# daooshee/ReReVST-Code

Measured on AMD Instinct MI355X. Metric: stylized frames/sec at 512x512, 1 style, higher is better.
Workload: dtype f32

## Files before the change

### rerevst-code_amd/csrc/conv_f43.h

```cpp
#pragma once
#include "conv_wino.h"

#ifndef F43_ABL
#define F43_ABL 0
#endif
#ifndef F43_SPAN
#define F43_SPAN 28
#endif

typedef float f32x2 __attribute__((ext_vector_type(2)));

struct F43Geo {
    static constexpr int NT = 256;
    static constexpr int NPOS = 36;
    static constexpr int RAW_ROW_BYTES = 4 * 9 * 32;
    static constexpr int RAW_PIECES = 34 * 4 * 9 * 2;
    static constexpr int RAW_IT = (RAW_PIECES + NT - 1) / NT;
    static constexpr int RAW_BYTES = RAW_IT * NT * 16;
    static constexpr int U_BYTES = NPOS * 32 * 8 * 4;
    static constexpr int U_IT = U_BYTES / 16 / NT;
    static constexpr int SMEM = 2 * RAW_BYTES + 2 * U_BYTES + WINO_PAR_BYTES;
};

__device__ __forceinline__ f32x2 p2sub(const f32x2 a, const f32x2 b) {
    f32x2 r;
    asm("v_pk_add_f32 %0, %1, %2 neg_lo:[0,1] neg_hi:[0,1]" : "=v"(r) : "v"(a), "v"(b));
    return r;
}
template <int IMM>
__device__ __forceinline__ f32x2 lds_rd64(unsigned addr) {
    static_assert(IMM >= 0 && IMM < 65536, "ds_read offset is a 16-bit unsigned immediate");
    f32x2 r;
    asm volatile("ds_read_b64 %0, %1 offset:%2" : "=v"(r) : "v"(addr), "i"(IMM));
    return r;
}

template <bool AG>
__device__ __forceinline__ void mfma_acc(f32x4& acc, const float a, const float b) {
    if constexpr (AG) asm volatile("v_mfma_f32_16x16x4_f32 %0, %1, %2, %0" : "+a"(acc) : "v"(a), "v"(b));
    else asm volatile("v_mfma_f32_16x16x4_f32 %0, %1, %2, %0" : "+v"(acc) : "v"(a), "v"(b));
}
template <bool AG>
__device__ __forceinline__ void mfma_zero(f32x4& acc, const float a, const float b) {
    if constexpr (AG) asm volatile("v_mfma_f32_16x16x4_f32 %0, %1, %2, 0" : "=a"(acc) : "v"(a), "v"(b));
    else asm volatile("v_mfma_f32_16x16x4_f32 %0, %1, %2, 0" : "=v"(acc) : "v"(a), "v"(b));
}

constexpr float F43_A = 0.75f, F43_B = 1.5f;
constexpr float F43_A2 = F43_A * F43_A, F43_B2 = F43_B * F43_B, F43_P = F43_A2 * F43_B2, F43_S = F43_A2 + F43_B2;
constexpr float F43_A3 = F43_A2 * F43_A, F43_B3 = F43_B2 * F43_B;
constexpr unsigned f43_bits(float f) { return __builtin_bit_cast(unsigned, f); }

struct F43Tmp { f32x2 a, b, c, f, g; };
struct F43K { unsigned long long b2, a2, p, s, a, b; };
__device__ __forceinline__ F43K f43_load_k() {
    F43K k;
    asm volatile("s_mov_b64 %0, %6\n\ts_mov_b64 %1, %7\n\ts_mov_b64 %2, %8\n\ts_mov_b64 %3, %9\n\ts_mov_b64 %4, %10\n\ts_mov_b64 %5, %11"
                 : "=s"(k.b2), "=s"(k.a2), "=s"(k.p), "=s"(k.s), "=s"(k.a), "=s"(k.b)
                 : "i"(f43_bits(F43_B2)), "i"(f43_bits(F43_A2)), "i"(f43_bits(F43_P)), "i"(f43_bits(F43_S)), "i"(f43_bits(F43_A)), "i"(f43_bits(F43_B)));
    return k;
}
template <bool NEG>
__device__ __forceinline__ void fmak3s(f32x2& r0, f32x2& r1, f32x2& r2, const f32x2 x0, const f32x2 x1, const f32x2 x2,
                                       const f32x2 c0, const f32x2 c1, const f32x2 c2, const unsigned long long ks) {
    if constexpr (NEG)
        asm volatile("v_pk_fma_f32 %0, %4, %3, %7 op_sel_hi:[1,0,1] neg_lo:[0,1,0] neg_hi:[0,1,0]\n\tv_pk_fma_f32 %1, %5, %3, %8 op_sel_hi:[1,0,1] neg_lo:[0,1,0] neg_hi:[0,1,0]\n\t"
                     "v_pk_fma_f32 %2, %6, %3, %9 op_sel_hi:[1,0,1] neg_lo:[0,1,0] neg_hi:[0,1,0]"
                     : "=&v"(r0), "=&v"(r1), "=&v"(r2) : "s"(ks), "v"(x0), "v"(x1), "v"(x2), "v"(c0), "v"(c1), "v"(c2));
    else
        asm volatile("v_pk_fma_f32 %0, %4, %3, %7 op_sel_hi:[1,0,1]\n\tv_pk_fma_f32 %1, %5, %3, %8 op_sel_hi:[1,0,1]\n\tv_pk_fma_f32 %2, %6, %3, %9 op_sel_hi:[1,0,1]"
                     : "=&v"(r0), "=&v"(r1), "=&v"(r2) : "s"(ks), "v"(x0), "v"(x1), "v"(x2), "v"(c0), "v"(c1), "v"(c2));
}
template <int LB, class LineFn>
__device__ __forceinline__ void f43_in3s(LineFn&& L, const F43K& k) {
    F43Tmp t[3];
    using N0 = std::integral_constant<int, LB>; using N1 = std::integral_constant<int, LB + 1>; using N2 = std::integral_constant<int, LB + 2>;
    using I0 = std::integral_constant<int, 0>; using I1 = std::integral_constant<int, 1>; using I2 = std::integral_constant<int, 2>;
    using I3 = std::integral_constant<int, 3>; using I4 = std::integral_constant<int, 4>; using I5 = std::integral_constant<int, 5>;
#define F43_D(J) L(N0{}, I##J{}), L(N1{}, I##J{}), L(N2{}, I##J{})
#define F43_T(M) t[0].M, t[1].M, t[2].M
    fmak3s<true>(F43_T(a), F43_D(2), F43_D(4), k.b2);
    fmak3s<true>(F43_T(b), F43_D(1), F43_D(3), k.b2);
    fmak3s<true>(F43_T(c), F43_D(2), F43_D(4), k.a2);
    fmak3s<true>(F43_T(f), F43_D(1), F43_D(3), k.a2);
    fmak3s<false>(F43_T(g), F43_D(0), F43_D(4), k.p);
    fmak3s<true>(F43_D(0), F43_D(2), F43_T(g), k.s);
    fmak3s<false>(F43_T(g), F43_D(1), F43_D(5), k.p);
    fmak3s<true>(F43_D(5), F43_D(3), F43_T(g), k.s);
    fmak3s<false>(F43_D(1), F43_T(b), F43_T(a), k.a);
    fmak3s<true>(F43_D(2), F43_T(b), F43_T(a), k.a);
    fmak3s<false>(F43_D(3), F43_T(f), F43_T(c), k.b);
    fmak3s<true>(F43_D(4), F43_T(f), F43_T(c), k.b);
#undef F43_D
#undef F43_T
}
__device__ __forceinline__ void f43_out(const f32x2 m0, const f32x2 m1, const f32x2 m2, const f32x2 m3, const f32x2 m4, const f32x2 m5,
                                        f32x2& y0, f32x2& y1, f32x2& y2, f32x2& y3) {
    f32x2 s1, d1, s2, d2;
    unsigned long long ks;
    asm volatile(
        "v_pk_add_f32 %[s1], %[m1], %[m2]\n\t"
        "v_pk_add_f32 %[d1], %[m1], %[m2] neg_lo:[0,1] neg_hi:[0,1]\n\t"
        "v_pk_add_f32 %[s2], %[m3], %[m4]\n\t"
        "v_pk_add_f32 %[d2], %[m3], %[m4] neg_lo:[0,1] neg_hi:[0,1]\n\t"
        "v_pk_add_f32 %[y0], %[m0], %[s1]\n\t"
        "s_mov_b64 %[k], %[ka]\n\t"
        "v_pk_mul_f32 %[y1], %[d1], %[k] op_sel_hi:[1,0]\n\t"
        "s_mov_b64 %[k], %[ka2]\n\t"
        "v_pk_mul_f32 %[y2], %[s1], %[k] op_sel_hi:[1,0]\n\t"
        "s_mov_b64 %[k], %[ka3]\n\t"
        "v_pk_fma_f32 %[y3], %[d1], %[k], %[m5] op_sel_hi:[1,0,1]\n\t"
        "v_pk_add_f32 %[y0], %[y0], %[s2]\n\t"
        "s_mov_b64 %[k], %[kb]\n\t"
        "v_pk_fma_f32 %[y1], %[d2], %[k], %[y1] op_sel_hi:[1,0,1]\n\t"
        "s_mov_b64 %[k], %[kb2]\n\t"
        "v_pk_fma_f32 %[y2], %[s2], %[k], %[y2] op_sel_hi:[1,0,1]\n\t"
        "s_mov_b64 %[k], %[kb3]\n\t"
        "v_pk_fma_f32 %[y3], %[d2], %[k], %[y3] op_sel_hi:[1,0,1]"
        : [y0] "=&v"(y0), [y1] "=&v"(y1), [y2] "=&v"(y2), [y3] "=&v"(y3), [s1] "=&v"(s1), [d1] "=&v"(d1), [s2] "=&v"(s2), [d2] "=&v"(d2), [k] "=&s"(ks)
        : [m0] "v"(m0), [m1] "v"(m1), [m2] "v"(m2), [m3] "v"(m3), [m4] "v"(m4), [m5] "v"(m5),
          [ka] "i"(f43_bits(F43_A)), [ka2] "i"(f43_bits(F43_A2)), [ka3] "i"(f43_bits(F43_A3)),
          [kb] "i"(f43_bits(F43_B)), [kb2] "i"(f43_bits(F43_B2)), [kb3] "i"(f43_bits(F43_B3)));
}

#ifndef P8_PAD
#define P8_PAD 6
#define P8_COL0 4
#endif
template <int EPI, int LAY = 0>
__global__ __launch_bounds__(256, 1) void conv_f43_k(const ConvP p) {
    static_assert(!(EPI & E_RES), "same-resolution residuals are not needed by the layers this kernel serves");
    constexpr bool INP8 = (LAY & 1) != 0, OUTP8 = (LAY & 2) != 0;
    const int WP = p.Wi + 2 + (INP8 ? P8_PAD : 0);
    using G = F43Geo;
    constexpr int ABL = F43_ABL;
    constexpr int RAW_BYTES = G::RAW_BYTES, U_BYTES = G::U_BYTES, NT = G::NT, NPOS = G::NPOS;
    extern __shared__ __attribute__((aligned(16))) char smem[];
    const int tid = threadIdx.x;
    const int wave = __builtin_amdgcn_readfirstlane(tid >> 6);
    const int lane = tid & 63, t = lane & 15, q = lane >> 4;
    const int tr = t >> 3, tc = t & 7;
    const int nchunks = p.Cin >> 3;
    const int n_ntiles = p.Cout >> 5;

    struct Item { int tx, ty, b, nt; };
    Item cur, nxt, dlt;
    {
        const int GD = gridDim.x, w = blockIdx.x;
        int pix, dpix;
        if (p.xcd_slabs) {
            const int PT = (GD >> 3) / n_ntiles;
            pix = (w & 7) * PT + (w >> 3) / n_ntiles; dpix = 8 * PT;
            cur.nt = (w >> 3) % n_ntiles; dlt.nt = 0;
        } else {
            cur.nt = w % n_ntiles; pix = w / n_ntiles;
            dlt.nt = GD % n_ntiles; dpix = GD / n_ntiles;
        }
        cur.tx = pix % p.tiles_x; cur.ty = (pix / p.tiles_x) % p.tiles_y; cur.b = pix / (p.tiles_x * p.tiles_y);
        dlt.tx = dpix % p.tiles_x; dlt.ty = (dpix / p.tiles_x) % p.tiles_y; dlt.b = dpix / (p.tiles_x * p.tiles_y);
    }
    auto advance = [&](const Item& a) {
        Item r = a;
        r.nt += dlt.nt;
        int carry = 0;
        if (r.nt >= n_ntiles) { r.nt -= n_ntiles; carry = 1; }
        r.tx += dlt.tx + carry;
        if (r.tx >= p.tiles_x) { r.tx -= p.tiles_x; r.ty += 1; }
        r.ty += dlt.ty;
        if (r.ty >= p.tiles_y) { r.ty -= p.tiles_y; r.b += 1; }
        r.b += dlt.b;
        return r;
    };
    const size_t img_floats = (size_t)(p.Hi + 2) * WP * p.Cin;
    auto in_of = [&](const Item& a) {
        return p.in + (size_t)a.b * img_floats + (size_t)(((a.ty + p.ty0) * 32) * WP + (a.tx + p.tx0) * 32 + (INP8 ? P8_COL0 - 1 : 0)) * (INP8 ? 8 : p.Cin);
    };
    const size_t plane_floats = (size_t)(p.Hi + 2) * WP * 8;
    auto lim_of = [&](const Item& a) {
        const long rows_left = (long)(p.Hi + 2) - (long)(a.ty + p.ty0) * 32;
        const long n = (rows_left * WP - (long)(a.tx + p.tx0) * 32 - (INP8 ? P8_COL0 - 1 : 0)) * (INP8 ? 8 : p.Cin) * 4;
        return (int)(n > 0x7fffffffL ? 0x7fffffffL : n);
    };
    auto w_of = [&](const Item& a) { return p.wpk + (size_t)a.nt * nchunks * (U_BYTES / 4); };
    int asrc[G::RAW_IT];
#pragma unroll
    for (int it = 0; it < G::RAW_IT; ++it) {
        int e = it * NT + tid;
        if (e >= G::RAW_PIECES) e = 0;
        const int half = e & 1, xd = (e >> 1) % 9, ph = ((e >> 1) / 9) & 3, y = (e >> 1) / 36;
        const int x = 4 * xd + ph, par = (y >> 2) & 1;
        asrc[it] = ((y * WP + x) * (INP8 ? 8 : p.Cin) + 4 * (half ^ par)) * 4;
        if (ABL & 64) asrc[it] = (it * NT + tid) * 16;
    }
    bool have = cur.b < p.B, have_nxt = false;
    const float* in_t = in_of(cur);
    const float* w_t = w_of(cur);
    int lim_t = lim_of(cur);
    const float* in_n = in_t;
    const float* w_n = w_t;
    int lim_n = lim_t;
    auto stage_u = [&](int chunk) {
        char* udst = smem + 2 * RAW_BYTES + (chunk & 1) * U_BYTES;
#pragma unroll
        for (int it = 0; it < G::U_IT; ++it) bufld16(w_t, udst + (it * NT + wave * 64) * 16, tid * 16, chunk * U_BYTES + it * NT * 16);
    };
    auto stage_raw = [&](int chunk) {
        char* rdst = smem + (chunk & 1) * RAW_BYTES;
        const rsrc_t rs = make_rsrc(INP8 ? in_t + chunk * plane_floats : in_t, lim_t);
#pragma unroll
        for (int it = 0; it < G::RAW_IT; ++it) bufld16_rs(rs, rdst + (it * NT + wave * 64) * 16, asrc[it], INP8 ? 0 : chunk * 32);
    };
    char* const par = smem + 2 * RAW_BYTES + 2 * U_BYTES;
    auto stage_params = [&](int ntile, int img) {
        if (wave < 2) {
            const int e = tid;
            const int row = e >> 3, col = (e & 7) * 4;
            const float* src = p.bias;
            int off = ntile * 32 + col;
            const int pb = img * p.par_bstride;
            if (row >= 1 && row <= 4) { src = (EPI & E_NORM1) ? p.n1 : p.bias; off += (EPI & E_NORM1) ? (row - 1) * p.Cout + pb : 0; }
            if (row >= 5 && row <= 8) { src = (EPI & E_NORM2) ? p.n2 : p.bias; off += (EPI & E_NORM2) ? (row - 5) * p.Cout + pb : 0; }
            if (row >= 9) { src = (EPI & E_NORM2) ? p.sty : p.bias; off += (EPI & E_NORM2) ? (row - 9) * p.Cout + pb : 0; }
            if (row > 10) { src = p.bias; off = ntile * 32; }
            glds16(src + off, par + wave * 1024);
        }
    };

    const unsigned lds0 = (unsigned)(size_t)(__attribute__((address_space(3))) char*)smem;
    const int y0 = 8 * wave + 4 * tr;
    const unsigned rawA = lds0 + y0 * G::RAW_ROW_BYTES + tc * 32 + ((q ^ (2 * (tr & 1))) << 3);
    const unsigned rawB = lds0 + y0 * G::RAW_ROW_BYTES + tc * 32 + ((q ^ (2 * ((tr & 1) ^ 1))) << 3);
    const unsigned offU = lds0 + 2 * RAW_BYTES + t * 64 + ((q ^ ((0 - (t >> 2)) & 3)) << 4);

    const unsigned lane_off = (unsigned)(((4 * (q >> 1)) * (p.W + 2) + 16 * (q & 1)) * p.Cout + 2 * t) * 4u;
#ifndef F43_NAG
#define F43_NAG 28
#endif
    constexpr int NAG = F43_NAG;
    f32x4 accA[NAG][2], accV[NPOS - NAG][2];
    int par_ntile = -1, par_img = -1;
    long long tl[6] = {0, 0, 0, 0, 0, 0}, tl_t = 0;
    auto tick = [&](int k) { if (ABL & 16) { const long long n = clock64(); tl[k] += n - tl_t; tl_t = n; } };
    f32x2 v[NPOS];
    f32x4 ur[2][6];
    auto full_transform = [&](f32x2 (&d)[NPOS]) {
        const F43K k = f43_load_k();
        auto col = [&](auto nc, auto jc) -> f32x2& { return d[decltype(nc)::value * 6 + decltype(jc)::value]; };
        auto row = [&](auto nc, auto jc) -> f32x2& { return d[decltype(jc)::value * 6 + decltype(nc)::value]; };
        f43_in3s<0>(col, k);
        f43_in3s<3>(col, k);
        f43_in3s<0>(row, k);
        f43_in3s<3>(row, k);
    };
    auto read_patch_col = [&](auto rbc, auto dxc) {
        constexpr int RB = decltype(rbc)::value, dx = decltype(dxc)::value;
        static_for([&](auto dyc) {
            constexpr int dy = decltype(dyc)::value;
            constexpr int off = RB + dy * G::RAW_ROW_BYTES + (dx & 3) * 288 + (dx >> 2) * 32;
            v[dx * 6 + dy] = lds_rd64<off>(dy < 4 ? rawA : rawB);
        }, std::make_integer_sequence<int, 6>{});
    };
    auto read_u_batch = [&](unsigned ub, auto bc, auto slotc) {
        constexpr int b = decltype(bc)::value, sl = decltype(slotc)::value;
        static_for([&](auto rc) {
            constexpr int r = decltype(rc)::value;
            ur[sl][r] = lds_rd128<(r * 6 + b) * 1024>(ub);
        }, std::make_integer_sequence<int, 6>{});
    };

    auto chunk_body = [&](int c, auto par_c, auto first_c, bool last) {
        constexpr int PAR = decltype(par_c)::value;
        constexpr bool FIRST = decltype(first_c)::value;
        const bool own_u = c + 1 < nchunks, own_r = c + 2 < nchunks;
        const rsrc_t rs_u = make_rsrc(own_u ? w_t : w_n);
        const int rchunk = own_r ? c + 2 : c + 2 - nchunks;
        const rsrc_t rs_r = make_rsrc(INP8 ? (own_r ? in_t : in_n) + rchunk * plane_floats : (own_r ? in_t : in_n), own_r ? lim_t : lim_n);
        const int usoff = own_u ? (c + 1) * U_BYTES : 0;
        const int rsoff = INP8 ? 0 : rchunk * 32;
        char* const udst = smem + 2 * RAW_BYTES + (1 - PAR) * U_BYTES;
        char* const rdst = smem + PAR * RAW_BYTES;
        const unsigned ub = offU + PAR * U_BYTES;
        const unsigned ubn = offU + (1 - PAR) * U_BYTES;
        using RBt = std::integral_constant<int, (1 - PAR) * RAW_BYTES>;
        static_for([&](auto bc) {
            constexpr int b = decltype(bc)::value;
            if constexpr (b <= 1) asm volatile("s_waitcnt lgkmcnt(0)" ::: "memory");
            else if (last) asm volatile("s_waitcnt lgkmcnt(0)" ::: "memory");
            else asm volatile("s_waitcnt lgkmcnt(6)" ::: "memory");
            if constexpr (b < 5) read_u_batch(ub, std::integral_constant<int, b + 1>{}, std::integral_constant<int, (b + 1) & 1>{});
            static_for([&](auto rc) {
                constexpr int r = decltype(rc)::value, pos = r * 6 + b;
                constexpr int step = b * 6 + r;
                auto dma_req = [&](auto nc) {
                    constexpr int n = decltype(nc)::value;
                    if constexpr (n < G::RAW_IT) bufld16_rs(rs_r, rdst + (n * NT + wave * 64) * 16, asrc[n], rsoff);
                    else if constexpr (n < G::RAW_IT + G::U_IT) bufld16_rs(rs_u, udst + ((n - G::RAW_IT) * NT + wave * 64) * 16, tid * 16, usoff + (n - G::RAW_IT) * NT * 16);
                };
                {
                    constexpr int SPAN = F43_SPAN, NREQ = G::RAW_IT + G::U_IT;
                    constexpr int n = (step * NREQ + SPAN - 1) / SPAN;
                    if constexpr (n < NREQ && (n * SPAN) / NREQ == step) { if (!(ABL & 1)) dma_req(std::integral_constant<int, n>{}); }
                }
                if constexpr (r == 3) {
                    if constexpr (b >= 1) { if (!last) read_patch_col(RBt{}, std::integral_constant<int, b - 1>{}); }
                }
                constexpr bool AG = pos < NAG;
                f32x4 (&ac)[2] = *[&]() -> f32x4 (*)[2] { if constexpr (AG) return &accA[pos]; else return &accV[pos - NAG]; }();
                const f32x2 vv = v[b * 6 + r];
                const f32x4 uu = ur[b & 1][r];
                if constexpr (FIRST) { mfma_zero<AG>(ac[0], vv[0], uu[0]); mfma_zero<AG>(ac[1], vv[0], uu[2]); }
                else { mfma_acc<AG>(ac[0], vv[0], uu[0]); mfma_acc<AG>(ac[1], vv[0], uu[2]); }
                mfma_acc<AG>(ac[0], vv[1], uu[1]);
                mfma_acc<AG>(ac[1], vv[1], uu[3]);
            }, std::make_integer_sequence<int, 6>{});
        }, std::make_integer_sequence<int, 6>{});
        if (!last) read_patch_col(RBt{}, std::integral_constant<int, 5>{});
        tick(1);
        if (!(ABL & 2)) asm volatile("s_waitcnt vmcnt(0) lgkmcnt(0)\n\ts_barrier" ::: "memory");
        else asm volatile("s_waitcnt lgkmcnt(0)" ::: "memory");
        tick(3);
        if (!last) {
            read_u_batch(ubn, std::integral_constant<int, 0>{}, std::integral_constant<int, 0>{});
            if (!(ABL & 8)) full_transform(v);
        }
        tick(5);
    };

    auto next_patch = [&]() {
        static_for([&](auto dxc) { read_patch_col(std::integral_constant<int, 0>{}, dxc); }, std::make_integer_sequence<int, 6>{});
        read_u_batch(offU, std::integral_constant<int, 0>{}, std::integral_constant<int, 0>{});
        if (!(ABL & 2)) asm volatile("s_waitcnt lgkmcnt(0)\n\ts_barrier" ::: "memory");
        else asm volatile("s_waitcnt lgkmcnt(0)" ::: "memory");
        if (!(ABL & 8)) full_transform(v);
    };
    if (have) {
        stage_raw(0);
        stage_u(0);
        stage_raw(1);
        stage_params(cur.nt, cur.b);
        par_ntile = cur.nt; par_img = cur.b;
        __syncthreads();
        next_patch();
        __syncthreads();
    }
    if (ABL & 16) tl_t = clock64();
    while (have) {
        const int e_y0 = (cur.ty + p.ty0) * 32, e_x0 = (cur.tx + p.tx0) * 32, e_b = cur.b, e_ntile = cur.nt;
        nxt = advance(cur);
        have_nxt = nxt.b < p.B;
        in_n = have_nxt ? in_of(nxt) : in_t;
        w_n = have_nxt ? w_of(nxt) : w_t;
        lim_n = have_nxt ? lim_of(nxt) : lim_t;
        if (par_ntile != e_ntile || (p.par_bstride != 0 && par_img != e_b)) {
            __syncthreads();
            stage_params(e_ntile, e_b);
            par_ntile = e_ntile; par_img = e_b;
        }
        tick(0);
        chunk_body(0, std::integral_constant<int, 0>{}, std::true_type{}, false);
        chunk_body(1, std::integral_constant<int, 1>{}, std::false_type{}, false);
        for (int c = 2; c < nchunks; c += 2) {
            chunk_body(c, std::integral_constant<int, 0>{}, std::false_type{}, false);
            chunk_body(c + 1, std::integral_constant<int, 1>{}, std::false_type{}, c + 2 == nchunks);
        }
        cur = nxt; have = have_nxt; in_t = in_n; w_t = w_n; lim_t = lim_n;
        asm volatile("s_nop 15\n\ts_nop 7");
        auto ACC = [&](int i, int nb) -> f32x4 { return i < NAG ? accA[i][nb] : accV[i - NAG][nb]; };
        if (ABL & 32) {
            f32x4 s = ACC(0, 0);
#pragma unroll
            for (int i = 0; i < NPOS; ++i)
#pragma unroll
                for (int nb = 0; nb < 2; ++nb) if (i || nb) s += ACC(i, nb);
            if (s[0] + s[1] + s[2] + s[3] == 123.456f) p.out[tid] = s[0];
            if (have) next_patch();
            continue;
        }
        const int mr = q >> 1, mc0 = 4 * (q & 1);
        const int yb = e_y0 + 8 * wave + 4 * mr, xb0 = e_x0 + 4 * mc0;
        constexpr bool POOL = (EPI & E_POOL) != 0;
        const int Ho = POOL ? (p.H >> 1) : p.H, Wo = POOL ? (p.W >> 1) : p.W;
        constexpr int OP = OUTP8 ? P8_PAD : 0;
        char* const sb = OUTP8 ? (char*)(p.out + (size_t)e_b * (size_t)(Ho + 2) * (Wo + 2 + OP) * p.Cout + (size_t)e_ntile * 4 * (size_t)(Ho + 2) * (Wo + 2 + OP) * 8 +
                                         ((size_t)((POOL ? (e_y0 >> 1) + 4 * wave : e_y0 + 8 * wave) + 1) * (Wo + 2 + OP) + (POOL ? (e_x0 >> 1) : e_x0) + P8_COL0) * 8)
                               : (char*)(p.out + (size_t)e_b * (size_t)(Ho + 2) * (Wo + 2) * p.Cout +
                                 ((size_t)((POOL ? (e_y0 >> 1) + 4 * wave : e_y0 + 8 * wave) + 1) * (Wo + 2) + (POOL ? (e_x0 >> 1) : e_x0) + 1) * p.Cout + e_ntile * 32);
        int rowb = (Wo + 2) * p.Cout * 4, pixb = p.Cout * 4;
        unsigned st_off = POOL ? (unsigned)(((2 * mr) * (Wo + 2) + 2 * mc0) * p.Cout + 2 * t) * 4u : lane_off;
        if constexpr (OUTP8) {
            const unsigned plane = (unsigned)(Ho + 2) * (Wo + 2 + OP) * 32u;
            rowb = (Wo + 2 + OP) * 32; pixb = 32;
            st_off = (POOL ? (unsigned)((2 * mr) * (Wo + 2 + OP) + 2 * mc0) : (unsigned)((4 * (q >> 1)) * (p.W + 2 + OP) + 16 * (q & 1))) * 32u + (unsigned)(t >> 2) * plane + (unsigned)(t & 3) * 8u;
        }
        const bool interior = e_y0 + 32 <= p.H && e_x0 + 32 <= p.W;
        const char* const pl = par + 8 * t;
        const f32x2 bias = *(const f32x2*)(pl);
        f32x2 n1m, n1r, n1lo, n1hi, n2m, n2r, n2lo, n2hi, smean, sstd;
        if constexpr ((EPI & E_NORM1) != 0) { n1m = *(const f32x2*)(pl + 128); n1r = *(const f32x2*)(pl + 256); n1lo = *(const f32x2*)(pl + 384); n1hi = *(const f32x2*)(pl + 512); }
        if constexpr ((EPI & E_NORM2) != 0) {
            n2m = *(const f32x2*)(pl + 640); n2r = *(const f32x2*)(pl + 768); n2lo = *(const f32x2*)(pl + 896); n2hi = *(const f32x2*)(pl + 1024);
            smean = *(const f32x2*)(pl + 1152); sstd = *(const f32x2*)(pl + 1280);
        }
        f32x2 rres[4][2][2];
        if constexpr ((EPI & E_RES_UPS) != 0) {
            const float* const res_b = p.res + (size_t)e_b * (size_t)(p.Hr + 2) * (p.Wr + 2) * p.Cout + e_ntile * 32 + 2 * t;
#pragma unroll
            for (int e = 0; e < 4; ++e)
#pragma unroll
                for (int a = 0; a < 2; ++a)
#pragma unroll
                    for (int b2 = 0; b2 < 2; ++b2) {
                        const bool in = (yb + 2 * a < p.H) && (xb0 + 4 * e + 2 * b2 < p.W);
                        const int pix = in ? (((yb >> 1) + a + 1) * (p.Wr + 2) + ((xb0 + 4 * e) >> 1) + b2 + 1) : 0;
                        rres[e][a][b2] = *(const f32x2*)(res_b + (size_t)pix * p.Cout);
                    }
        }
        float lrk = 0.2f;
        asm volatile("" : "+s"(lrk));
        const f32x2 lrk2 = {lrk, lrk};
#pragma unroll
        for (int e = 0; e < 4; ++e) {
            auto PR = [&](int i) -> f32x2 { return f32x2{ACC(i, 0)[e], ACC(i, 1)[e]}; };
            f32x2 T[6][4];
#pragma unroll
            for (int r = 0; r < 6; ++r) {
                f43_out(PR(r * 6 + 0), PR(r * 6 + 1), PR(r * 6 + 2), PR(r * 6 + 3), PR(r * 6 + 4), PR(r * 6 + 5), T[r][0], T[r][1], T[r][2], T[r][3]);
                __builtin_amdgcn_sched_barrier(0);
            }
            f32x2 pool_prev[2];
#pragma unroll
            for (int j = 0; j < 4; ++j) {
                f32x2 o[4];
                f43_out(T[0][j], T[1][j], T[2][j], T[3][j], T[4][j], T[5][j], o[0], o[1], o[2], o[3]);
#pragma unroll
                for (int i = 0; i < 4; ++i) o[i] = o[i] + bias;
                if (EPI & E_RELU) {
#pragma unroll
                    for (int i = 0; i < 4; ++i) o[i] = f32x2{fmaxf(o[i][0], 0.f), fmaxf(o[i][1], 0.f)};
                }
                if (EPI & E_LRELU) {
#pragma unroll
                    for (int i = 0; i < 4; ++i) { const f32x2 s2 = o[i] * lrk2; o[i] = f32x2{fmaxf(o[i][0], s2[0]), fmaxf(o[i][1], s2[1])}; }
                }
                auto norm_clamp = [&](const f32x2 m, const f32x2 r, const f32x2 lo, const f32x2 hi) {
#pragma unroll
                    for (int i = 0; i < 4; ++i) o[i] = p2sub(o[i], m) * r;
#pragma unroll
                    for (int i = 0; i < 4; ++i) o[i] = f32x2{med3(o[i][0], lo[0], hi[0]), med3(o[i][1], lo[1], hi[1])};
                };
                if constexpr ((EPI & E_NORM1) != 0) norm_clamp(n1m, n1r, n1lo, n1hi);
                if constexpr ((EPI & E_RES_UPS) != 0) {
#pragma unroll
                    for (int i = 0; i < 4; ++i) o[i] = o[i] + rres[e][i >> 1][j >> 1];
                }
                if constexpr ((EPI & E_NORM2) != 0) {
                    norm_clamp(n2m, n2r, n2lo, n2hi);
#pragma unroll
                    for (int i = 0; i < 4; ++i) o[i] = __builtin_elementwise_fma(o[i], sstd, smean);
                }
                if constexpr (POOL) {
                    f32x2 m2[2];
#pragma unroll
                    for (int a = 0; a < 2; ++a) m2[a] = f32x2{fmaxf(o[2 * a][0], o[2 * a + 1][0]), fmaxf(o[2 * a][1], o[2 * a + 1][1])};
                    if ((j & 1) == 0) { pool_prev[0] = m2[0]; pool_prev[1] = m2[1]; continue; }
#pragma unroll
                    for (int a = 0; a < 2; ++a) m2[a] = f32x2{fmaxf(m2[a][0], pool_prev[a][0]), fmaxf(m2[a][1], pool_prev[a][1])};
                    char* const dst = sb + (2 * e + (j >> 1)) * pixb + st_off;
                    if (ABL & 4) { if (m2[0][0] == 123.456f) *(float*)dst = m2[0][0] + m2[1][0]; }
                    else if (interior) {
                        *(f32x2*)(dst) = m2[0]; *(f32x2*)(dst + rowb) = m2[1];
                    } else {
#pragma unroll
                        for (int a = 0; a < 2; ++a)
                            if ((yb >> 1) + a < Ho && ((xb0 + 4 * e) >> 1) + (j >> 1) < Wo) *(f32x2*)(dst + a * rowb) = m2[a];
                    }
                } else {
                    char* const dst = sb + (4 * e + j) * pixb + st_off;
                    if (ABL & 4) { if (o[0][0] == 123.456f) *(float*)dst = o[0][0] + o[1][0] + o[2][0] + o[3][0]; }
                    else if (interior) {
#pragma unroll
                        for (int i = 0; i < 4; ++i) *(f32x2*)(dst + i * rowb) = o[i];
                    } else {
#pragma unroll
                        for (int i = 0; i < 4; ++i)
                            if (yb + i < p.H && xb0 + 4 * e + j < p.W) *(f32x2*)(dst + i * rowb) = o[i];
                    }
                }
            }
        }
        tick(4);
        if (have) next_patch();
        tick(5);
    }
    if ((ABL & 16) && lane == 0) {
#pragma unroll
        for (int k = 0; k < 6; ++k) p.dbg[(blockIdx.x * 4 + wave) * 6 + k] = tl[k];
    }
}

__global__ void pack_f43_k(const float* __restrict__ w, float* __restrict__ dst, int Cout, int Cin) {
    const size_t total = (size_t)Cout * Cin * 36;
    for (size_t i = blockIdx.x * (size_t)blockDim.x + threadIdx.x; i < total; i += (size_t)gridDim.x * blockDim.x) {
        size_t r = i;
        const int fl = (int)(r & 3); r >>= 2;
        const int slot = (int)(r & 3); r >>= 2;
        const int row = (int)(r & 15); r >>= 4;
        const int pos = (int)(r % 36); r /= 36;
        const int nchunks = Cin / 8;
        const int chunk = (int)(r % nchunks); r /= nchunks;
        const int n_tile = (int)r;
        const int pair = slot ^ ((0 - (row >> 2)) & 3);
        const int co = n_tile * 32 + 2 * row + (fl >> 1), ci = chunk * 8 + 2 * pair + (fl & 1);
        const float* g = w + ((size_t)co * Cin + ci) * 9;
        const int pr = pos / 6, pc = pos % 6;
        auto G3 = [](int rw, double g0, double g1, double g2) -> double {
            const double A = (double)F43_A, B = (double)F43_B;
            const double pt[5] = {0.0, A, -A, B, -B};
            if (rw == 5) return g2;
            double N = 1.0;
            for (int l = 0; l < 5; ++l) if (l != rw) N *= pt[rw] - pt[l];
            return (g0 + pt[rw] * g1 + pt[rw] * pt[rw] * g2) / N;
        };
        double rowv[3];
#pragma unroll
        for (int kx = 0; kx < 3; ++kx) rowv[kx] = G3(pr, g[0 * 3 + kx], g[1 * 3 + kx], g[2 * 3 + kx]);
        dst[i] = (float)G3(pc, rowv[0], rowv[1], rowv[2]);
    }
}
```

### rerevst-code_amd/csrc/conv_mfma.h

```cpp
#pragma once
#include <hip/hip_runtime.h>
#include <stdint.h>

typedef float f32x16 __attribute__((ext_vector_type(16)));
typedef float f32x4 __attribute__((ext_vector_type(4)));

enum {
    E_RELU = 1,
    E_LRELU = 2,
    E_NORM1 = 4,
    E_RES = 8,
    E_RES_UPS = 16,
    E_NORM2 = 32,
    E_POOL = 64
};

struct ConvP {
    const float* in;
    int Hi, Wi, Cin;
    float* out;
    int H, W, Cout;
    int B;
    int in_bstride0;
    const float* wpk;
    const float* bias;
    const float* n1;
    const float* res;
    int Hr, Wr;
    const float* n2;
    const float* sty;
    int tiles_x, tiles_y;
    int xcd_slabs;
    float* sc_out;
    int ty0, tx0;
    long long* dbg;
    int cstride;
    int cin_slab_step;
    int par_bstride, bias_bstride;
    long long w_bstride;
    int out_p8;
};

template <int BN>
struct WaveCfg {
    static constexpr int WAVES_N = (BN >= 64) ? 2 : 1;
    static constexpr int WAVES_M = 4 / WAVES_N;
    static constexpr int WN_SUB = BN / 32 / WAVES_N;
    static constexpr int WM_SUB = 4 / WAVES_M;
};

__device__ __forceinline__ void glds16(const float* src, char* lds_wave_base) {
    __builtin_amdgcn_global_load_lds((const __attribute__((address_space(1))) void*)src,
                                     (__attribute__((address_space(3))) void*)lds_wave_base, 16, 0, 0);
}

__device__ __forceinline__ void bufld16(const void* base, char* lds_wave_base, int voff, int soff) {
#if defined(__HIP_DEVICE_COMPILE__)
    __amdgpu_buffer_rsrc_t rs = __builtin_amdgcn_make_buffer_rsrc((void*)base, 0, 0x7fffffff, 0x00020000);
    __builtin_amdgcn_raw_ptr_buffer_load_lds(rs, (__attribute__((address_space(3))) void*)lds_wave_base, 16, voff, soff, 0, 0);
#endif
}

#if defined(__HIP_DEVICE_COMPILE__)
typedef __amdgpu_buffer_rsrc_t rsrc_t;
#else
struct rsrc_t {};
#endif
__device__ __forceinline__ rsrc_t make_rsrc(const void* base, int num_records = 0x7fffffff) {
#if defined(__HIP_DEVICE_COMPILE__)
    return __builtin_amdgcn_make_buffer_rsrc((void*)base, 0, num_records, 0x00020000);
#else
    return rsrc_t{};
#endif
}
__device__ __forceinline__ void bufld16_rs(rsrc_t rs, char* lds_wave_base, int voff, int soff) {
#if defined(__HIP_DEVICE_COMPILE__)
    __builtin_amdgcn_raw_ptr_buffer_load_lds(rs, (__attribute__((address_space(3))) void*)lds_wave_base, 16, voff, soff, 0, 0);
#endif
}

template <int BN, int TAPS, int EPI, int ABL = 0, int MSUB = 0, int LD = 1>
__global__ __launch_bounds__(256) void conv_mfma_k(const ConvP p) {
    using WC = WaveCfg<BN>;
    constexpr int WM_SUB = MSUB ? MSUB : WC::WM_SUB;
    constexpr int TROWS = WC::WAVES_M * WM_SUB * 2;
    constexpr int HWD = (TAPS == 1) ? 16 : 18;
    constexpr int HHT = (TAPS == 1) ? TROWS : TROWS + 2;
    constexpr int NPIX = HHT * HWD;
    constexpr int A_ITERS = (NPIX * 4 + 255) / 256;
    constexpr int A_BYTES = A_ITERS * 256 * 16;
    constexpr int B_PIECES = BN * 4;
    constexpr int B_ITERS = (B_PIECES + 255) / 256;
    constexpr int B_BYTES = BN * 64;
    __shared__ __attribute__((aligned(16))) char smem[2 * A_BYTES + 2 * B_BYTES];

    const int tid = threadIdx.x;
    const int wave = __builtin_amdgcn_readfirstlane(tid >> 6);
    const int lane = tid & 63, h = lane >> 5, l31 = lane & 31;
    const int wave_m = wave % WC::WAVES_M, wave_n = wave / WC::WAVES_M;

    int bx = blockIdx.x;
    const int tx = bx % p.tiles_x;
    bx /= p.tiles_x;
    const int ty = bx % p.tiles_y;
    const int b = bx / p.tiles_y;
    const int n_tile = blockIdx.y;
    const int y0 = ty * TROWS, x0 = tx * 16;
    const int nchunks = p.Cin >> 4;

    const float* in_b = p.in + (size_t)(p.in_bstride0 ? b : 0) * (size_t)(p.Hi + 2) * (p.Wi + 2) * p.Cin;
    const int ys = (TAPS == 1) ? y0 : y0 - 1;
    const int xs = (TAPS == 1) ? x0 : x0 - 1;
    int asrc[A_ITERS];
#pragma unroll
    for (int it = 0; it < A_ITERS; ++it) {
        const int e = it * 256 + tid;
        int pp = e >> 2;
        const int qq = e & 3;
        if (pp >= NPIX) pp = 0;
        const int hy = pp / HWD, hx = pp - hy * HWD;
        asrc[it] = (hy * (p.Wi + 2) + hx) * p.Cin + 4 * (qq ^ ((pp >> 2) & 3));
    }
    const float* in_t = in_b + ((size_t)(ys + 1) * (p.Wi + 2) + (xs + 1)) * p.Cin;
    const float* wsrc = p.wpk + (size_t)n_tile * nchunks * TAPS * (BN * 16) + tid * 4;

    const float* w_tile = p.wpk + (size_t)n_tile * nchunks * TAPS * (BN * 16);
    auto stage = [&](int chunk, int tap, int step) {
        char* bdst = smem + 2 * A_BYTES + (step & 1) * B_BYTES;
        const float* wb = wsrc + (size_t)(chunk * TAPS + tap) * (BN * 16);
#pragma unroll
        for (int it = 0; it < B_ITERS; ++it) {
            if (B_PIECES >= 256 || wave * 64 < B_PIECES) {
                if (LD == 1)
                    bufld16(w_tile, bdst + (it * 256 + wave * 64) * 16, tid * 16, (chunk * TAPS + tap) * (BN * 64) + it * 4096);
                else
                    glds16(wb + it * 1024, bdst + (it * 256 + wave * 64) * 16);
            }
        }
        if (tap == 0) {
            char* adst = smem + (chunk & 1) * A_BYTES;
            const float* ab = in_t + chunk * 16;
#pragma unroll
            for (int it = 0; it < A_ITERS; ++it) {
                if (LD == 1)
                    bufld16(in_t, adst + (it * 256 + wave * 64) * 16, asrc[it] * 4, chunk * 64);
                else
                    glds16(ab + asrc[it], adst + (it * 256 + wave * 64) * 16);
            }
        }
    };

    const int r_ = l31 >> 4, c_ = l31 & 15;
    int offB[WC::WN_SUB][2];
#pragma unroll
    for (int ns = 0; ns < WC::WN_SUB; ++ns) {
        const int jj = (wave_n * WC::WN_SUB + ns) * 32 + l31;
#pragma unroll
        for (int g = 0; g < 2; ++g) offB[ns][g] = jj * 64 + ((((2 * g + h) ^ ((jj >> 2) & 3))) << 4);
    }

    f32x16 acc[WM_SUB][WC::WN_SUB];
#pragma unroll
    for (int ms = 0; ms < WM_SUB; ++ms)
#pragma unroll
        for (int ns = 0; ns < WC::WN_SUB; ++ns)
#pragma unroll
            for (int r = 0; r < 16; ++r) acc[ms][ns][r] = 0.f;

    long long t_start = 0, t_loop = 0;
    if (ABL & 16) t_start = clock64();
    stage(0, 0, 0);
    int step = 0;
    for (int chunk = 0; chunk < nchunks; ++chunk) {
        const char* abuf = smem + (chunk & 1) * A_BYTES;
#pragma unroll
        for (int tap = 0; tap < TAPS; ++tap, ++step) {
            if (!(ABL & 2) || step == 0) __syncthreads();
            if (!(ABL & 1)) {
                if (tap + 1 < TAPS)
                    stage(chunk, tap + 1, step + 1);
                else if (chunk + 1 < nchunks)
                    stage(chunk + 1, 0, step + 1);
            }
            const char* bbuf = smem + 2 * A_BYTES + (step & 1) * B_BYTES;
            const int ky = tap / 3, kx = tap - ky * 3;
            int offA[WM_SUB];
#pragma unroll
            for (int ms = 0; ms < WM_SUB; ++ms) {
                const int msg = wave_m * WM_SUB + ms;
                int pp;
                if (TAPS == 1)
                    pp = (2 * msg + r_) * HWD + c_;
                else
                    pp = (2 * msg + r_ + ky) * HWD + c_ + kx;
                offA[ms] = pp * 64 + ((h ^ ((pp >> 2) & 3)) << 4);
            }
#pragma unroll
            for (int g = 0; g < 2; ++g) {
                f32x4 a[WM_SUB], bb[WC::WN_SUB];
#pragma unroll
                for (int ms = 0; ms < WM_SUB; ++ms) a[ms] = *(const f32x4*)(abuf + (offA[ms] ^ (g << 5)));
#pragma unroll
                for (int ns = 0; ns < WC::WN_SUB; ++ns) bb[ns] = *(const f32x4*)(bbuf + offB[ns][g]);
#pragma unroll
                for (int s = 0; s < 4; ++s)
#pragma unroll
                    for (int ms = 0; ms < WM_SUB; ++ms)
#pragma unroll
                        for (int ns = 0; ns < WC::WN_SUB; ++ns)
                            acc[ms][ns] = __builtin_amdgcn_mfma_f32_32x32x2f32(bb[ns][s], a[ms][s], acc[ms][ns], 0, 0, 0);
            }
        }
    }

    if (ABL & 16) t_loop = clock64();
    const int Ho = (EPI & E_POOL) ? (p.H >> 1) : p.H, Wo = (EPI & E_POOL) ? (p.W >> 1) : p.W;
    float* out_b = p.out + (size_t)b * (size_t)(Ho + 2) * (Wo + 2) * p.Cout;
    const float* res_b = nullptr;
    if (EPI & (E_RES | E_RES_UPS)) res_b = p.res + (size_t)b * (size_t)(p.Hr + 2) * (p.Wr + 2) * p.Cout;
#pragma unroll
    for (int ns = 0; ns < WC::WN_SUB; ++ns) {
#pragma unroll
        for (int cg = 0; cg < 4; ++cg) {
            const int co = n_tile * BN + (wave_n * WC::WN_SUB + ns) * 32 + 8 * cg + 4 * h;
            const f32x4 bias = *(const f32x4*)(p.bias + co);
            f32x4 m1, r1, lo1, hi1, m2, r2, lo2, hi2, smean, sstd;
            if (EPI & E_NORM1) {
                m1 = *(const f32x4*)(p.n1 + co); r1 = *(const f32x4*)(p.n1 + p.Cout + co);
                lo1 = *(const f32x4*)(p.n1 + 2 * p.Cout + co); hi1 = *(const f32x4*)(p.n1 + 3 * p.Cout + co);
            }
            if (EPI & E_NORM2) {
                m2 = *(const f32x4*)(p.n2 + co); r2 = *(const f32x4*)(p.n2 + p.Cout + co);
                lo2 = *(const f32x4*)(p.n2 + 2 * p.Cout + co); hi2 = *(const f32x4*)(p.n2 + 3 * p.Cout + co);
                smean = *(const f32x4*)(p.sty + co); sstd = *(const f32x4*)(p.sty + p.Cout + co);
            }
#pragma unroll
            for (int ms = 0; ms < WM_SUB; ++ms) {
                const int msg = wave_m * WM_SUB + ms;
                const int y = y0 + 2 * msg + r_, x = x0 + c_;
                const bool valid = (y < p.H) && (x < p.W);
                f32x4 v;
#pragma unroll
                for (int e = 0; e < 4; ++e) {
                    float t = acc[ms][ns][4 * cg + e] + bias[e];
                    if (EPI & E_RELU) t = fmaxf(t, 0.f);
                    if (EPI & E_LRELU) t = (t >= 0.f) ? t : t * 0.2f;
                    if (EPI & E_NORM1) {
                        t = (t - m1[e]) * r1[e];
                        t = fminf(hi1[e], fmaxf(lo1[e], t));
                    }
                    v[e] = t;
                }
                if (EPI & (E_RES | E_RES_UPS)) {
                    if (valid) {
                        const int ry = (EPI & E_RES_UPS) ? (y >> 1) : y, rx = (EPI & E_RES_UPS) ? (x >> 1) : x;
                        v += *(const f32x4*)(res_b + ((ry + 1) * (p.Wr + 2) + rx + 1) * p.Cout + co);
                    }
                }
                if (EPI & E_NORM2) {
#pragma unroll
                    for (int e = 0; e < 4; ++e) {
                        float t = (v[e] - m2[e]) * r2[e];
                        t = fminf(hi2[e], fmaxf(lo2[e], t));
                        v[e] = t * sstd[e] + smean[e];
                    }
                }
                if (EPI & E_POOL) {
#pragma unroll
                    for (int e = 0; e < 4; ++e) {
                        float t = v[e];
                        t = fmaxf(t, __shfl_xor(t, 1));
                        t = fmaxf(t, __shfl_xor(t, 16));
                        v[e] = t;
                    }
                    const int y2 = (y0 >> 1) + msg, x2 = (x0 + c_) >> 1;
                    if (r_ == 0 && !(c_ & 1) && y2 < Ho && x2 < Wo) {
                        if (ABL & 4) { if (v[0] == 123.456f) out_b[co] = v[0]; }
                        else *(f32x4*)(out_b + ((y2 + 1) * (Wo + 2) + x2 + 1) * p.Cout + co) = v;
                    }
                } else if (valid) {
                    if (ABL & 4) { if (v[0] == 123.456f) out_b[co] = v[0]; }
                    else *(f32x4*)(out_b + ((y + 1) * (p.W + 2) + x + 1) * p.Cout + co) = v;
                }
            }
        }
    }
    if (ABL & 16) {
        const long long t_issued = clock64();
        __builtin_amdgcn_s_waitcnt(0);
        const long long t_end = clock64();
        if (lane == 0) {
            long long* dbg = p.dbg;
            const int wg = (blockIdx.y * gridDim.x + blockIdx.x) * 4 + wave;
            dbg[wg * 4 + 0] = t_start; dbg[wg * 4 + 1] = t_loop; dbg[wg * 4 + 2] = t_issued; dbg[wg * 4 + 3] = t_end;
        }
    }
}
```

### rerevst-code_amd/csrc/conv_ups5.h

```cpp
#pragma once

struct Ups5Tab {
    static constexpr int G2[5][3] = {{2, 0, 0}, {1, 1, 1}, {-1, -1, 1}, {-1, 1, 1}, {0, 0, 2}};
    static constexpr int BT4[4][4] = {{1, 0, -1, 0}, {0, 1, 1, 0}, {0, -1, 1, 0}, {0, -1, 0, 1}};
    static constexpr int AT[4][5] = {{1, 1, 0, -1, 0}, {0, 1, 1, 0, 0}, {0, 1, 0, 1, 0}, {0, 1, -1, 0, 1}};
    static constexpr int DS[5] = {0, 1, 2, 2, 3};
};
template <int T, int R>
constexpr int ups5_coef(int k) { return T == 0 ? Ups5Tab::BT4[R][k] : Ups5Tab::AT[R][k]; }
template <int T, int R, int N>
__device__ __forceinline__ f32x4 ups5_comb(const f32x4 (&x)[N]) {
    constexpr int F = [] { for (int k = 0; k < N; ++k) if (ups5_coef<T, R>(k) == 1) return k; return -1; }();
    static_assert(F >= 0, "every row has a +1 coefficient");
    f32x4 r = x[F];
    static_for([&](auto kc) {
        constexpr int k = decltype(kc)::value;
        constexpr int c = ups5_coef<T, R>(k);
        static_assert(c == 0 || c == 1 || c == -1, "0 / +-1 coefficients");
        if constexpr (k != F && c == 1) r = e4add(r, x[k]);
        else if constexpr (c == -1) r = f4sub(r, x[k]);
    }, std::make_integer_sequence<int, N>{});
    return r;
}

struct Ups5Geo {
    static constexpr int NT = 256, NB = 2;
    static constexpr int NPOS = 29;
    static constexpr int NUB = 26;
    static constexpr int NPIECE = 16;
    static constexpr int HALO = 18, HALF = 18 * 9;
    static constexpr int PIECES = HALO * HALO * 4;
    static constexpr int RAW_IT = (PIECES + NT - 1) / NT;
    static constexpr int RAW_BYTES = RAW_IT * NT * 16;
    static constexpr int U_BYTES = NUB * 32 * 16 * 4;
    static constexpr int U_IT = U_BYTES / 16 / NT;
    static_assert(U_IT * NT * 16 == U_BYTES, "U image is a whole number of LDS-DMA rounds");
    static constexpr int SMEM = 2 * RAW_BYTES + 2 * U_BYTES + WINO_PAR_BYTES;
    static_assert(SMEM <= 160 * 1024, "LDS");
    static constexpr int OCC = 1;
    static constexpr int vidx(int i) { return i < 25 ? Ups5Tab::DS[i % 5] * 4 + Ups5Tab::DS[i / 5] : (i == 25 ? 5 : i == 26 ? 9 : i == 27 ? 6 : 10); }
    static constexpr int issued(int j) { return (j + 2 < NUB ? 2 : 0) + (j < NPIECE ? 1 : 0); }
    static constexpr int younger(int i) {
        return i == 0 ? 2 + issued(0) : i == 1 ? issued(0) + issued(1) : (i - 2 < NPIECE ? 1 : 0) + issued(i - 1) + issued(i);
    }
    static constexpr int col_iter(int dx) { return 4 * dx + 6; }
    static constexpr int row_iter(int r) { return col_iter(3) + 1 + r; }
};
static_assert(Ups5Geo::row_iter(3) < Ups5Geo::NPOS, "next chunk transformed inside the MFMA loop");

template <int EPI, int PERIMG>
__device__ __forceinline__ void conv_ups5_body(const ConvP& p) {
    static_assert(!(EPI & (E_POOL | E_RES | E_RES_UPS | E_NORM2)), "conv1 epilogues only: bias, activation, saved-stat normalise");
    using G = Ups5Geo;
    constexpr int RAW_BYTES = G::RAW_BYTES, U_BYTES = G::U_BYTES, NT = G::NT, NB = G::NB, NPOS = G::NPOS, NUB = G::NUB;
    extern __shared__ __attribute__((aligned(16))) char smem[];
    const int tid = threadIdx.x;
    const int wave = __builtin_amdgcn_readfirstlane(tid >> 6);
    const int lane = tid & 63, t = lane & 15, q = lane >> 4;
    const int tr = t >> 3, tc = t & 7;
    const int tg = wave;
    const int nchunks = p.Cin >> 4;
    const int n_ntiles = p.Cout >> 5;

    struct Item { int tx, ty, b, nt; };
    Item cur, nxt, dlt;
    {
        const int GD = gridDim.x, w = blockIdx.x;
        int pix, dpix;
        if (p.xcd_slabs) {
            const int PT = (GD >> 3) / n_ntiles;
            pix = (w & 7) * PT + (w >> 3) / n_ntiles; dpix = 8 * PT;
            cur.nt = (w >> 3) % n_ntiles; dlt.nt = 0;
        } else {
            cur.nt = w % n_ntiles; pix = w / n_ntiles;
            dlt.nt = GD % n_ntiles; dpix = GD / n_ntiles;
        }
        cur.tx = pix % p.tiles_x; cur.ty = (pix / p.tiles_x) % p.tiles_y; cur.b = pix / (p.tiles_x * p.tiles_y);
        dlt.tx = dpix % p.tiles_x; dlt.ty = (dpix / p.tiles_x) % p.tiles_y; dlt.b = dpix / (p.tiles_x * p.tiles_y);
    }
    auto advance = [&](const Item& a) {
        Item r = a;
        r.nt += dlt.nt;
        int carry = 0;
        if (r.nt >= n_ntiles) { r.nt -= n_ntiles; carry = 1; }
        r.tx += dlt.tx + carry;
        if (r.tx >= p.tiles_x) { r.tx -= p.tiles_x; r.ty += 1; }
        r.ty += dlt.ty;
        if (r.ty >= p.tiles_y) { r.ty -= p.tiles_y; r.b += 1; }
        r.b += dlt.b;
        return r;
    };
    auto in_of = [&](const Item& a) {
        return p.in + (size_t)a.b * (size_t)(p.Hi + 2) * (p.Wi + 2) * p.Cin + (size_t)(((a.ty + p.ty0) * 16) * (p.Wi + 2) + (a.tx + p.tx0) * 16) * p.Cin;
    };
    auto w_of = [&](const Item& a) { return p.wpk + (size_t)a.nt * nchunks * (NUB * 32 * 16); };
    int asrc[G::RAW_IT];
#pragma unroll
    for (int it = 0; it < G::RAW_IT; ++it) {
        const int e = it * NT + tid;
        int P = e >> 2;
        const int qq = e & 3;
        if (P >= G::HALO * G::HALO) P = 0;
        const int hf = P >= G::HALF, rem = P - hf * G::HALF;
        const int hy = rem / 9, hx = 2 * (rem - hy * 9) + hf;
        asrc[it] = ((hy * (p.Wi + 2) + hx) * p.Cin + 4 * (qq ^ ((hx >> 1) & 3))) * 4;
    }
    const int raw_last_num = ((G::RAW_IT - 1) * NT + wave * 64 < G::PIECES) ? 0x7fffffff : 0;
    bool have = cur.b < p.B, have_nxt = false;
    const float* in_t = in_of(cur);
    const float* w_t = w_of(cur);
    const float* in_n = in_t;
    const float* w_n = w_t;
    auto stage_u = [&](int chunk) {
        char* udst = smem + 2 * RAW_BYTES + (chunk & 1) * U_BYTES;
#pragma unroll
        for (int it = 0; it < G::U_IT; ++it) bufld16(w_t, udst + (it * NT + wave * 64) * 16, tid * 16, chunk * U_BYTES + it * NT * 16);
    };
    auto stage_raw = [&](int chunk) {
        char* rdst = smem + (chunk & 1) * RAW_BYTES;
#pragma unroll
        for (int it = 0; it < G::RAW_IT; ++it)
            if (it * NT + wave * 64 < G::PIECES) bufld16(in_t, rdst + (it * NT + wave * 64) * 16, asrc[it], chunk * 64);
    };
    char* const par = smem + 2 * RAW_BYTES + 2 * U_BYTES;
    auto stage_params = [&](int ntile, int img) {
        if (wave < 2) {
            const int e = tid;
            const int row = e >> 3, col = (e & 7) * 4;
            const float* src = p.bias;
            const int pb = PERIMG ? img * p.par_bstride : 0;
            int off = ntile * 32 + col;
            if (row >= 1 && row <= 4) { src = (EPI & E_NORM1) ? p.n1 : p.bias; off = (EPI & E_NORM1) ? ntile * 32 + col + pb + (row - 1) * p.Cout : off; }
            if (row > 4) { src = p.bias; off = ntile * 32; }
            glds16(src + off, par + wave * 1024);
        }
    };

    const unsigned lds0 = (unsigned)(size_t)(__attribute__((address_space(3))) char*)smem;
    unsigned offD[4];
#pragma unroll
    for (int dx = 0; dx < 4; ++dx) {
        const int hy = 4 * tg + 2 * tr, hx = 2 * tc + dx;
        const int P = (hx & 1) * G::HALF + hy * 9 + (hx >> 1);
        offD[dx] = lds0 + P * 64 + ((q ^ ((hx >> 1) & 3)) << 4);
    }
    const unsigned offU = lds0 + 2 * RAW_BYTES + t * 64 + ((q ^ ((0 - (t >> 2)) & 3)) << 4);
    const unsigned offU1 = offU + U_BYTES;

    f32x4 acc[NPOS][NB];
    f32x4 va[16], vb[16];
    auto pass = [](f32x4& x0, f32x4& x1, f32x4& x2, f32x4& x3) {
        const f32x4 a[4] = {x0, x1, x2, x3};
        x0 = ups5_comb<0, 0>(a); x1 = ups5_comb<0, 1>(a); x2 = ups5_comb<0, 2>(a); x3 = ups5_comb<0, 3>(a);
    };
    auto col_pass = [&](f32x4 (&d)[16], int dx) { pass(d[dx * 4 + 0], d[dx * 4 + 1], d[dx * 4 + 2], d[dx * 4 + 3]); };
    auto row_pass = [&](f32x4 (&d)[16], int r) { pass(d[0 * 4 + r], d[1 * 4 + r], d[2 * 4 + r], d[3 * 4 + r]); };

    auto chunk_body = [&](int c, auto par_c, auto first_c, f32x4 (&vcur)[16], f32x4 (&vnext)[16]) {
        constexpr int PAR = decltype(par_c)::value;
        constexpr bool FIRST = decltype(first_c)::value;
        const bool own_u = c + 1 < nchunks, own_r = c + 2 < nchunks;
        const rsrc_t rs_u = make_rsrc(own_u ? w_t : w_n);
        const rsrc_t rs_r = make_rsrc(own_r ? in_t : in_n);
        const rsrc_t rs_rl = make_rsrc(own_r ? in_t : in_n, raw_last_num);
        const int usoff = own_u ? (c + 1) * U_BYTES : 0;
        const int rsoff = (own_r ? c + 2 : c + 2 - nchunks) * 64;
        char* const udst = smem + 2 * RAW_BYTES + (1 - PAR) * U_BYTES;
        char* const rdst = smem + PAR * RAW_BYTES;
        const unsigned ub = PAR ? offU1 : offU;
        constexpr int RB = (1 - PAR) * RAW_BYTES;
        f32x4 u[4][NB];
        f32x4 (&d)[16] = vnext;
        u[0][0] = lds_rd128<0>(ub);
        u[0][1] = lds_rd128<1024>(ub);
        u[1][0] = lds_rd128<2048>(ub);
        u[1][1] = lds_rd128<2048 + 1024>(ub);
        static_for([&](auto ic) {
            constexpr int i = decltype(ic)::value;
            if constexpr (i + 2 < NUB) {
                u[(i + 2) & 3][0] = lds_rd128<(i + 2) * 2048>(ub);
                u[(i + 2) & 3][1] = lds_rd128<(i + 2) * 2048 + 1024>(ub);
            }
            if constexpr (i < 16) d[i] = lds_rd128<RB + (i & 3) * 576>(offD[i >> 2]);
            constexpr int US = (i < NUB ? i : NUB - 1) & 3;
            if constexpr (i < NUB) {
                constexpr int cdx = (i - 6) / 4;
                if constexpr (i >= 6 && (i - 6) % 4 == 0 && cdx < 4) {
                    static_assert(G::col_iter(cdx) == i, "column release schedule");
                    asm volatile("s_waitcnt lgkmcnt(%6)" : "+v"(d[cdx * 4 + 0]), "+v"(d[cdx * 4 + 1]), "+v"(d[cdx * 4 + 2]), "+v"(d[cdx * 4 + 3]),
                                 "+v"(u[US][0]), "+v"(u[US][1]) : "i"(G::younger(i)));
                } else {
                    lds_release2<G::younger(i)>(u[US][0], u[US][1]);
                }
            }
            __builtin_amdgcn_sched_barrier(0);
            if constexpr (i < G::U_IT) bufld16_rs(rs_u, udst + (i * NT + wave * 64) * 16, tid * 16, usoff + i * NT * 16);
            if constexpr (i < G::RAW_IT) bufld16_rs(i == G::RAW_IT - 1 ? rs_rl : rs_r, rdst + (i * NT + wave * 64) * 16, asrc[i], rsoff);
            const f32x4 vv = vcur[G::vidx(i)];
#pragma unroll
            for (int s = 0; s < 4; ++s)
#pragma unroll
                for (int nb = 0; nb < NB; ++nb)
                    acc[i][nb] = __builtin_amdgcn_mfma_f32_16x16x4f32(u[US][nb][s], vv[s], (FIRST && s == 0) ? f32x4{0.f, 0.f, 0.f, 0.f} : acc[i][nb], 0, 0, 0);
            static_for([&](auto xc) {
                constexpr int k = decltype(xc)::value;
                if constexpr (G::col_iter(k) == i) col_pass(d, k);
                if constexpr (G::row_iter(k) == i) row_pass(d, k);
            }, std::make_integer_sequence<int, 4>{});
        }, std::make_integer_sequence<int, NPOS>{});
    };

    int par_ntile = -1, par_img = -1;
    if (have) {
        stage_raw(0);
        stage_u(0);
        stage_raw(1);
        stage_params(cur.nt, cur.b);
        par_ntile = cur.nt; par_img = cur.b;
        __syncthreads();
#pragma unroll
        for (int k = 0; k < 16; ++k) va[k] = *(const f32x4*)(smem + (offD[k >> 2] - lds0) + (k & 3) * 576);
#pragma unroll
        for (int dx = 0; dx < 4; ++dx) col_pass(va, dx);
#pragma unroll
        for (int r = 0; r < 4; ++r) row_pass(va, r);
        __syncthreads();
    }
    while (have) {
        const int e_y0 = (cur.ty + p.ty0) * 32, e_x0 = (cur.tx + p.tx0) * 32, e_b = cur.b, e_ntile = cur.nt;
        nxt = advance(cur);
        have_nxt = nxt.b < p.B;
        in_n = have_nxt ? in_of(nxt) : in_t;
        w_n = have_nxt ? w_of(nxt) : w_t;
        if (par_ntile != e_ntile || (PERIMG && par_img != e_b)) {
            __syncthreads();
            stage_params(e_ntile, e_b);
            par_ntile = e_ntile; par_img = e_b;
        }
        chunk_body(0, std::integral_constant<int, 0>{}, std::true_type{}, va, vb);
        __syncthreads();
        chunk_body(1, std::integral_constant<int, 1>{}, std::false_type{}, vb, va);
        __syncthreads();
        for (int c = 2; c < nchunks; c += 2) {
            chunk_body(c, std::integral_constant<int, 0>{}, std::false_type{}, va, vb);
            __syncthreads();
            chunk_body(c + 1, std::integral_constant<int, 1>{}, std::false_type{}, vb, va);
            __syncthreads();
        }
        cur = nxt; have = have_nxt; in_t = in_n; w_t = w_n;

        float* out_b = p.out + (size_t)e_b * (size_t)(p.H + 2) * (p.W + 2 + (p.out_p8 ? 6 : 0)) * p.Cout;
        const int yb = e_y0 + 8 * tg + 4 * tr, xb = e_x0 + 4 * tc;
        {
            const int ly0 = yb >> 1, lx0 = xb >> 1;
            float* sc_b = p.sc_out + (size_t)e_b * (size_t)(p.Hi + 2) * (p.Wi + 2) * p.Cout;
#pragma unroll
            for (int nb = 0; nb < NB; ++nb) {
                const f32x4 s0 = f4sub(acc[25][nb], acc[27][nb]), s1 = e4add(acc[25][nb], acc[27][nb]);
                const f32x4 t0 = f4sub(acc[26][nb], acc[28][nb]), t1 = e4add(acc[26][nb], acc[28][nb]);
                const f32x4 sc[2][2] = {{f4sub(s0, t0), e4add(s0, t0)}, {f4sub(s1, t1), e4add(s1, t1)}};
#pragma unroll
                for (int a = 0; a < 2; ++a)
#pragma unroll
                    for (int b = 0; b < 2; ++b) {
                        const int ly = ly0 + a, lx = lx0 + b;
                        if (ly < p.Hi && lx < p.Wi)
                            *(f32x4*)(sc_b + ((size_t)(ly + 1) * (p.Wi + 2) + lx + 1) * p.Cout + e_ntile * 32 + nb * 16 + 4 * q) = sc[a][b];
                    }
            }
        }
#pragma unroll
        for (int nb = 0; nb < NB; ++nb) {
            const int co = e_ntile * 32 + nb * 16 + 4 * q;
            f32x4 T[5][4];
#pragma unroll
            for (int r = 0; r < 5; ++r) {
                const f32x4 m[5] = {acc[r * 5 + 0][nb], acc[r * 5 + 1][nb], acc[r * 5 + 2][nb], acc[r * 5 + 3][nb], acc[r * 5 + 4][nb]};
                T[r][0] = ups5_comb<1, 0>(m); T[r][1] = ups5_comb<1, 1>(m); T[r][2] = ups5_comb<1, 2>(m); T[r][3] = ups5_comb<1, 3>(m);
            }
            f32x4 Y[4][4];
#pragma unroll
            for (int j = 0; j < 4; ++j) {
                const f32x4 tj[5] = {T[0][j], T[1][j], T[2][j], T[3][j], T[4][j]};
                Y[0][j] = ups5_comb<1, 0>(tj); Y[1][j] = ups5_comb<1, 1>(tj); Y[2][j] = ups5_comb<1, 2>(tj); Y[3][j] = ups5_comb<1, 3>(tj);
            }
            const char* pl = par + (nb * 16 + 4 * q) * 4;
            const f32x4 bias = *(const f32x4*)(pl);
            f32x4 m1, r1, lo1, hi1;
            if (EPI & E_NORM1) {
                m1 = *(const f32x4*)(pl + 128); r1 = *(const f32x4*)(pl + 256);
                lo1 = *(const f32x4*)(pl + 384); hi1 = *(const f32x4*)(pl + 512);
            }
#pragma unroll
            for (int i = 0; i < 4; ++i)
#pragma unroll
                for (int j = 0; j < 4; ++j) {
                    const int y = yb + i, x = xb + j;
                    f32x4 o = e4add(Y[i][j], bias);
                    if (EPI & E_RELU) o = f4relu(o);
                    if (EPI & E_LRELU) o = f4lrelu(o);
                    if (EPI & E_NORM1) o = f4norm_clamp(o, m1, r1, lo1, hi1);
                    if (y < p.H && x < p.W) {
                        if (p.out_p8) *(f32x4*)(out_b + (size_t)(co >> 3) * ((size_t)(p.H + 2) * (p.W + 8) * 8) + ((size_t)(y + 1) * (p.W + 8) + x + 4) * 8 + (co & 7)) = o;
                        else *(f32x4*)(out_b + ((size_t)(y + 1) * (p.W + 2) + x + 1) * p.Cout + co) = o;
                    }
                }
        }
    }
    asm volatile("s_waitcnt vmcnt(0)" ::: "memory");
}

__global__ void pack_ups5_k(const float* __restrict__ w, const float* __restrict__ wsc, float* __restrict__ dst, int Cout, int Cin) {
    constexpr int CH = 16, NUB = Ups5Geo::NUB;
    const size_t total = (size_t)Cout * Cin * NUB;
    for (size_t i = blockIdx.x * (size_t)blockDim.x + threadIdx.x; i < total; i += (size_t)gridDim.x * blockDim.x) {
        size_t r = i;
        const int cl = (int)(r % CH); r /= CH;
        const int j = r & 31; r >>= 5;
        const int pos = (int)(r % NUB); r /= NUB;
        const int nchunks = Cin / CH;
        const int chunk = r % nchunks; r /= nchunks;
        const int n_tile = (int)r;
        const int e = cl & 3, qs = cl >> 2;
        const int qq = qs ^ ((0 - (j >> 2)) & 3);
        const int co = n_tile * 32 + j, ci = chunk * CH + qq * 4 + e;
        if (pos == 25) { dst[i] = wsc[(size_t)co * Cin + ci] * 0.25f; continue; }
        const float* g = w + ((size_t)co * Cin + ci) * 9;
        auto G5 = [](int row, double g0, double g1, double g2) {
            return 0.5 * (Ups5Tab::G2[row][0] * g0 + Ups5Tab::G2[row][1] * g1 + Ups5Tab::G2[row][2] * g2);
        };
        const int pr = pos / 5, pc = pos % 5;
        double rowv[3];
#pragma unroll
        for (int kx = 0; kx < 3; ++kx) rowv[kx] = G5(pr, g[0 * 3 + kx], g[1 * 3 + kx], g[2 * 3 + kx]);
        dst[i] = (float)G5(pc, rowv[0], rowv[1], rowv[2]);
    }
}
```

### rerevst-code_amd/csrc/conv_wino.h

```cpp
#pragma once
#include <hip/hip_runtime.h>
#include <stdint.h>
#include <utility>
#include <type_traits>
#include "conv_mfma.h"

#define WINO_PAR_BYTES 2048

template <int NW, int UPS>
struct WinoGeo {
    static constexpr int NT = NW * 64;
    static constexpr int NB = NW == 8 ? 1 : 2;
    static constexpr int NP = UPS ? 9 : 16;
    static constexpr int NPU = NP;
    static constexpr int PW = UPS ? 3 : 4;
    static constexpr int NPIECE = PW * PW;
    static constexpr int PPI = UPS ? 3 : 2;
    static constexpr int TIN = UPS ? 8 : 16;
    static constexpr int HALO = UPS ? 10 : 18;
    static constexpr int HALF = 18 * 9;
    static constexpr int PIECES = HALO * HALO * 4;
    static constexpr int RAW_IT = (PIECES + NT - 1) / NT;
    static constexpr int RAW_BYTES = RAW_IT * NT * 16;
    static constexpr int U_BYTES = NPU * 32 * 16 * 4;
    static constexpr int U_PIECES = U_BYTES / 16;
    static constexpr int U_IT = (U_PIECES + NT - 1) / NT;
    static constexpr int U_LDS = U_IT * NT * 16;
    static constexpr int SMEM = 2 * RAW_BYTES + 2 * U_LDS + WINO_PAR_BYTES;
    static constexpr int OCC = (UPS && NW == 4) ? 2 : 1;
    static constexpr int col_iter(int dx) { return (dx * PW + PW - 1) / PPI + 3; }
    static constexpr int row_iter(int r) { return col_iter(PW - 1) + 1 + r; }
    static constexpr int pieces_in(int i) { return i < 0 ? 0 : (NPIECE - i * PPI <= 0 ? 0 : (NPIECE - i * PPI < PPI ? NPIECE - i * PPI : PPI)); }
    static constexpr int issued(int i) { return (i + 2 < NPU ? NB : 0) + pieces_in(i); }
    static constexpr int younger(int i) {
        return i == 0 ? NB + issued(0) : i == 1 ? issued(0) + issued(1) : pieces_in(i - 2) + issued(i - 1) + issued(i);
    }
};

template <int IMM>
__device__ __forceinline__ f32x4 lds_rd128(unsigned addr) {
    static_assert(IMM >= 0 && IMM < 65536, "ds_read offset is a 16-bit unsigned immediate");
    f32x4 r;
    asm volatile("ds_read_b128 %0, %1 offset:%2" : "=v"(r) : "v"(addr), "i"(IMM));
    return r;
}
template <int N>
__device__ __forceinline__ void lds_release1(f32x4& a) {
    asm volatile("s_waitcnt lgkmcnt(%1)" : "+v"(a) : "i"(N));
}
template <int N>
__device__ __forceinline__ void lds_release2(f32x4& a, f32x4& b) {
    asm volatile("s_waitcnt lgkmcnt(%2)" : "+v"(a), "+v"(b) : "i"(N));
}
template <int N>
__device__ __forceinline__ void lds_release3(f32x4& a, f32x4& b, f32x4& c) {
    asm volatile("s_waitcnt lgkmcnt(%3)" : "+v"(a), "+v"(b), "+v"(c) : "i"(N));
}
template <int N>
__device__ __forceinline__ void lds_release4(f32x4& a, f32x4& b, f32x4& c, f32x4& d) {
    asm volatile("s_waitcnt lgkmcnt(%4)" : "+v"(a), "+v"(b), "+v"(c), "+v"(d) : "i"(N));
}

__device__ __forceinline__ f32x4 f4sub(const f32x4 a, const f32x4 b) {
    typedef float f32x2 __attribute__((ext_vector_type(2)));
    f32x2 lo, hi;
    asm("v_pk_add_f32 %0, %1, %2 neg_lo:[0,1] neg_hi:[0,1]" : "=v"(lo) : "v"(__builtin_shufflevector(a, a, 0, 1)), "v"(__builtin_shufflevector(b, b, 0, 1)));
    asm("v_pk_add_f32 %0, %1, %2 neg_lo:[0,1] neg_hi:[0,1]" : "=v"(hi) : "v"(__builtin_shufflevector(a, a, 2, 3)), "v"(__builtin_shufflevector(b, b, 2, 3)));
    return __builtin_shufflevector(lo, hi, 0, 1, 2, 3);
}

__device__ __forceinline__ f32x4 f4add(const f32x4 a, const f32x4 b) {
    typedef float f32x2 __attribute__((ext_vector_type(2)));
    f32x2 lo, hi;
    asm("v_pk_add_f32 %0, %1, %2" : "=v"(lo) : "v"(__builtin_shufflevector(a, a, 0, 1)), "v"(__builtin_shufflevector(b, b, 0, 1)));
    asm("v_pk_add_f32 %0, %1, %2" : "=v"(hi) : "v"(__builtin_shufflevector(a, a, 2, 3)), "v"(__builtin_shufflevector(b, b, 2, 3)));
    return __builtin_shufflevector(lo, hi, 0, 1, 2, 3);
}

typedef float f32x2_t __attribute__((ext_vector_type(2)));
#define F4_LO(v) __builtin_shufflevector(v, v, 0, 1)
#define F4_HI(v) __builtin_shufflevector(v, v, 2, 3)
__device__ __forceinline__ f32x4 e4add(const f32x4 a, const f32x4 b) {
    const f32x2_t lo = F4_LO(a) + F4_LO(b), hi = F4_HI(a) + F4_HI(b);
    return __builtin_shufflevector(lo, hi, 0, 1, 2, 3);
}
__device__ __forceinline__ f32x4 e4mul(const f32x4 a, const f32x4 b) {
    const f32x2_t lo = F4_LO(a) * F4_LO(b), hi = F4_HI(a) * F4_HI(b);
    return __builtin_shufflevector(lo, hi, 0, 1, 2, 3);
}
__device__ __forceinline__ f32x4 e4fma(const f32x4 a, const f32x4 b, const f32x4 c) {
    const f32x2_t lo = __builtin_elementwise_fma(F4_LO(a), F4_LO(b), F4_LO(c)), hi = __builtin_elementwise_fma(F4_HI(a), F4_HI(b), F4_HI(c));
    return __builtin_shufflevector(lo, hi, 0, 1, 2, 3);
}
__device__ __forceinline__ float med3(float v, float lo, float hi) {
    float r;
    asm("v_med3_f32 %0, %1, %2, %3" : "=v"(r) : "v"(v), "v"(lo), "v"(hi));
    return r;
}
__device__ __forceinline__ f32x4 f4relu(f32x4 v) {
#pragma unroll
    for (int e = 0; e < 4; ++e) v[e] = fmaxf(v[e], 0.f);
    return v;
}
__device__ __forceinline__ f32x4 f4lrelu(const f32x4 v) {
    float k = 0.2f;
    asm volatile("" : "+s"(k));
    const f32x2_t k2 = {k, k};
    const f32x2_t lo = F4_LO(v) * k2, hi = F4_HI(v) * k2;
    const f32x4 s = __builtin_shufflevector(lo, hi, 0, 1, 2, 3);
    f32x4 r;
#pragma unroll
    for (int e = 0; e < 4; ++e) r[e] = fmaxf(v[e], s[e]);
    return r;
}
__device__ __forceinline__ f32x4 f4norm_clamp(const f32x4 v, const f32x4 m, const f32x4 r, const f32x4 lo, const f32x4 hi) {
    const f32x4 n = e4mul(f4sub(v, m), r);
    f32x4 o;
#pragma unroll
    for (int e = 0; e < 4; ++e) o[e] = med3(n[e], lo[e], hi[e]);
    return o;
}

template <class F, int... I>
__device__ __forceinline__ void static_for(F&& f, std::integer_sequence<int, I...>) {
    (f(std::integral_constant<int, I>{}), ...);
}

#include "conv_ups5.h"

template <int EPI, int ABL, int NW, int UPS, int PERIMG>
__device__ __forceinline__ void conv_upw_body(const ConvP& p) {
    static_assert(!(EPI & E_POOL), "no pooling behind an upsample");
    using G = WinoGeo<NW, UPS>;
    constexpr int NPU = G::NPU;
    constexpr int RAW_BYTES = G::RAW_BYTES, U_BYTES = G::U_BYTES, U_LDS = G::U_LDS, NT = G::NT, NB = G::NB, NP = G::NP, PW = G::PW, NPIECE = G::NPIECE;
    extern __shared__ __attribute__((aligned(16))) char smem[];
    const int tid = threadIdx.x;
    const int wave = __builtin_amdgcn_readfirstlane(tid >> 6);
    const int lane = tid & 63, t = lane & 15, q = lane >> 4;
    const int tr = t >> 3, tc = t & 7;
    const int tg = wave;
    const int nchunks = p.Cin >> 4;
    const int n_ntiles = p.Cout >> 5;

    struct Item { int tx, ty, b, nt; };
    Item cur, nxt, dlt;
    {
        const int GD = gridDim.x, w = blockIdx.x;
        int pix, dpix;
        if (p.xcd_slabs) {
            const int PT = (GD >> 3) / n_ntiles;
            pix = (w & 7) * PT + (w >> 3) / n_ntiles; dpix = 8 * PT;
            cur.nt = (w >> 3) % n_ntiles; dlt.nt = 0;
        } else {
            cur.nt = w % n_ntiles; pix = w / n_ntiles;
            dlt.nt = GD % n_ntiles; dpix = GD / n_ntiles;
        }
        cur.tx = pix % p.tiles_x; cur.ty = (pix / p.tiles_x) % p.tiles_y; cur.b = pix / (p.tiles_x * p.tiles_y);
        dlt.tx = dpix % p.tiles_x; dlt.ty = (dpix / p.tiles_x) % p.tiles_y; dlt.b = dpix / (p.tiles_x * p.tiles_y);
    }
    auto advance = [&](const Item& a) {
        Item r = a;
        r.nt += dlt.nt;
        int carry = 0;
        if (r.nt >= n_ntiles) { r.nt -= n_ntiles; carry = 1; }
        r.tx += dlt.tx + carry;
        if (r.tx >= p.tiles_x) { r.tx -= p.tiles_x; r.ty += 1; }
        r.ty += dlt.ty;
        if (r.ty >= p.tiles_y) { r.ty -= p.tiles_y; r.b += 1; }
        r.b += dlt.b;
        return r;
    };
    auto in_of = [&](const Item& a) {
        return p.in + (size_t)a.b * (size_t)(p.Hi + 2) * (p.Wi + 2) * p.Cin + (size_t)(((a.ty + p.ty0) * G::TIN) * (p.Wi + 2) + (a.tx + p.tx0) * G::TIN) * p.Cin;
    };
    auto w_of = [&](const Item& a) { return p.wpk + (size_t)a.nt * nchunks * (NPU * 32 * 16); };
    int asrc[G::RAW_IT];
#pragma unroll
    for (int it = 0; it < G::RAW_IT; ++it) {
        const int e = it * NT + tid;
        int P = e >> 2;
        const int qq = e & 3;
        if (P >= G::HALO * G::HALO) P = 0;
        const int hy = P / 10, hx = P - hy * 10, swz = hx & 3;
        asrc[it] = ((hy * (p.Wi + 2) + hx) * p.Cin + 4 * (qq ^ swz)) * 4;
    }
    const int raw_last_num = ((G::RAW_IT - 1) * NT + wave * 64 < G::PIECES) ? 0x7fffffff : 0;
    const int u_last_num = ((G::U_IT - 1) * NT + wave * 64 < G::U_PIECES) ? 0x7fffffff : 0;
    bool have = cur.b < p.B, have_nxt = false;
    const float* in_t = in_of(cur);
    const float* w_t = w_of(cur);
    const float* in_n = in_t;
    const float* w_n = w_t;
    auto stage_u = [&](int chunk) {
        char* udst = smem + 2 * RAW_BYTES + (chunk & 1) * U_LDS;
#pragma unroll
        for (int it = 0; it < G::U_IT; ++it)
            if (it * NT + wave * 64 < G::U_PIECES) bufld16(w_t, udst + (it * NT + wave * 64) * 16, tid * 16, chunk * U_BYTES + it * NT * 16);
    };
    auto stage_raw = [&](int chunk) {
        char* rdst = smem + (chunk & 1) * RAW_BYTES;
#pragma unroll
        for (int it = 0; it < G::RAW_IT; ++it)
            if (it * NT + wave * 64 < G::PIECES) bufld16(in_t, rdst + (it * NT + wave * 64) * 16, asrc[it], chunk * 64);
    };

    char* const par = smem + 2 * RAW_BYTES + 2 * U_LDS;
    auto stage_params = [&](int ntile, int img) {
        if (wave < 2) {
            const int e = tid;
            const int row = e >> 3, col = (e & 7) * 4;
            const float* src = p.bias;
            const int pb = PERIMG ? img * p.par_bstride : 0;
            int off = ntile * 32 + col;
            if (row >= 1 && row <= 4) { src = (EPI & E_NORM1) ? p.n1 : p.bias; off = (EPI & E_NORM1) ? ntile * 32 + col + pb + (row - 1) * p.Cout : off; }
            if (row >= 5 && row <= 8) { src = (EPI & E_NORM2) ? p.n2 : p.bias; off = (EPI & E_NORM2) ? ntile * 32 + col + pb + (row - 5) * p.Cout : off; }
            if (row >= 9) { src = (EPI & E_NORM2) ? p.sty : p.bias; off = (EPI & E_NORM2) ? ntile * 32 + col + pb + (row - 9) * p.Cout : off; }
            if (row > 10) { src = p.bias; off = ntile * 32; }
            glds16(src + off, par + wave * 1024);
        }
    };

    const unsigned lds0 = (unsigned)(size_t)(__attribute__((address_space(3))) char*)smem;
    unsigned offD[NPIECE];
#pragma unroll
    for (int dx = 0; dx < PW; ++dx)
#pragma unroll
        for (int dy = 0; dy < PW; ++dy) {
            const int hy = 2 * tg + tr + dy, hx = tc + dx;
            offD[dx * PW + dy] = lds0 + (hy * 10 + hx) * 64 + ((q ^ (hx & 3)) << 4);
        }
    const unsigned offU = lds0 + 2 * RAW_BYTES + t * 64 + ((q ^ ((0 - (t >> 2)) & 3)) << 4);
    const unsigned offU1 = offU + U_LDS;

    f32x4 acc[NPU][NB];
    f32x4 va[NPIECE], vb[NPIECE];
    auto pass = [](f32x4& d0, f32x4& d1, f32x4& d2) {
        const f32x4 a0 = d0, a1 = d1, a2 = d2;
        d0 = a1; d1 = f4sub(a0, a1); d2 = f4sub(a2, a1);
    };
    auto col_pass = [&](f32x4 (&d)[NPIECE], int dx) {
        pass(d[dx * PW + 0], d[dx * PW + 1], d[dx * PW + 2]);
    };
    auto row_pass = [&](f32x4 (&d)[NPIECE], int r) {
        pass(d[0 * PW + r], d[1 * PW + r], d[2 * PW + r]);
    };

    auto chunk_body = [&](int c, auto par_c, auto first_c, f32x4 (&vcur)[NPIECE], f32x4 (&vnext)[NPIECE]) {
        constexpr int PAR = decltype(par_c)::value;
        constexpr bool FIRST = decltype(first_c)::value;
        const bool own_u = c + 1 < nchunks, own_r = c + 2 < nchunks;
        const rsrc_t rs_u = make_rsrc(own_u ? w_t : w_n);
        const rsrc_t rs_ul = make_rsrc(own_u ? w_t : w_n, u_last_num);
        const rsrc_t rs_r = make_rsrc(own_r ? in_t : in_n);
        const rsrc_t rs_rl = make_rsrc(own_r ? in_t : in_n, raw_last_num);
        const int usoff = own_u ? (c + 1) * U_BYTES : 0;
        const int rsoff = (own_r ? c + 2 : c + 2 - nchunks) * 64;
        char* const udst = smem + 2 * RAW_BYTES + (1 - PAR) * U_LDS;
        char* const rdst = smem + PAR * RAW_BYTES;
        if (ABL & 128) {
            f32x4 u01[2] = {vcur[0], vcur[1]};
#pragma unroll
            for (int i = 0; i < NPU; ++i) {
                const f32x4 vv = vcur[i];
#pragma unroll
                for (int s = 0; s < 4; ++s)
#pragma unroll
                    for (int nb = 0; nb < NB; ++nb)
                        acc[i][nb] = __builtin_amdgcn_mfma_f32_16x16x4f32(u01[nb][s], vv[s], (FIRST && s == 0) ? f32x4{0.f, 0.f, 0.f, 0.f} : acc[i][nb], 0, 0, 0);
            }
#pragma unroll
            for (int i = 0; i < NPIECE; ++i) vnext[i] = vcur[i];
            return;
        }
        const unsigned ub = PAR ? offU1 : offU;
        constexpr int RB = (1 - PAR) * RAW_BYTES;
        f32x4 u[4][NB];
        f32x4 (&d)[NPIECE] = vnext;
        u[0][0] = lds_rd128<0>(ub);
        u[0][1] = lds_rd128<1024>(ub);
        u[1][0] = lds_rd128<2048>(ub);
        u[1][1] = lds_rd128<2048 + 1024>(ub);
        static_for([&](auto ic) {
            constexpr int i = decltype(ic)::value;
            if constexpr (i + 2 < NPU) {
                u[(i + 2) & 3][0] = lds_rd128<(i + 2) * 2048>(ub);
                u[(i + 2) & 3][1] = lds_rd128<(i + 2) * 2048 + 1024>(ub);
            }
            static_for([&](auto kc) {
                constexpr int pc = i * G::PPI + decltype(kc)::value;
                if constexpr (pc < NPIECE) d[pc] = lds_rd128<RB>(offD[pc]);
            }, std::make_integer_sequence<int, G::PPI>{});
            constexpr int cdx = i - 3;
            static_assert(G::col_iter(0) == 3 && G::col_iter(PW - 1) == PW + 2, "column release schedule");
            if constexpr (cdx >= 0 && cdx < PW) {
                asm volatile("s_waitcnt lgkmcnt(%5)" : "+v"(d[cdx * 3 + 0]), "+v"(d[cdx * 3 + 1]), "+v"(d[cdx * 3 + 2]), "+v"(u[i & 3][0]), "+v"(u[i & 3][1]) : "i"(G::younger(i)));
            } else {
                lds_release2<G::younger(i)>(u[i & 3][0], u[i & 3][1]);
            }
            __builtin_amdgcn_sched_barrier(0);
            if (!(ABL & 1)) {
                {
                    if constexpr (i < G::U_IT) bufld16_rs(i == G::U_IT - 1 ? rs_ul : rs_u, udst + (i * NT + wave * 64) * 16, tid * 16, usoff + i * NT * 16);
                    if constexpr (i < G::RAW_IT) bufld16_rs(i == G::RAW_IT - 1 ? rs_rl : rs_r, rdst + (i * NT + wave * 64) * 16, asrc[i], rsoff);
                }
            }
            const f32x4 vv = vcur[(i % PW) * PW + i / PW];
#pragma unroll
            for (int s = 0; s < 4; ++s)
#pragma unroll
                for (int nb = 0; nb < NB; ++nb)
                    acc[i][nb] = __builtin_amdgcn_mfma_f32_16x16x4f32(u[i & 3][nb][s], vv[s], (FIRST && s == 0) ? f32x4{0.f, 0.f, 0.f, 0.f} : acc[i][nb], 0, 0, 0);
            static_for([&](auto xc) {
                constexpr int k = decltype(xc)::value;
                if constexpr (G::col_iter(k) == i) col_pass(d, k);
                if constexpr (G::row_iter(k) == i) row_pass(d, k);
            }, std::make_integer_sequence<int, PW>{});
        }, std::make_integer_sequence<int, NPU>{});
    };

    int par_ntile = -1, par_img = -1;
    long long tl[6] = {0, 0, 0, 0, 0, 0}, tl_t = 0;
    auto tick = [&](int k) { if (ABL & 16) { const long long n = clock64(); tl[k] += n - tl_t; tl_t = n; } };
    if (ABL & 16) tl_t = clock64();
    if (have) {
        stage_raw(0);
        stage_u(0);
        stage_raw(1);
        stage_params(cur.nt, cur.b);
        par_ntile = cur.nt; par_img = cur.b;
        __syncthreads();
#pragma unroll
        for (int k = 0; k < NPIECE; ++k) va[k] = *(const f32x4*)(smem + (offD[k] - lds0));
#pragma unroll
        for (int dx = 0; dx < PW; ++dx) col_pass(va, dx);
#pragma unroll
        for (int r = 0; r < PW; ++r) row_pass(va, r);
        __syncthreads();
    }
    while (have) {
        const int e_y0 = (cur.ty + p.ty0) * 16, e_x0 = (cur.tx + p.tx0) * 16, e_b = cur.b, e_ntile = cur.nt;
        nxt = advance(cur);
        have_nxt = nxt.b < p.B;
        in_n = have_nxt ? in_of(nxt) : in_t;
        w_n = have_nxt ? w_of(nxt) : w_t;
        if (par_ntile != e_ntile || (PERIMG && par_img != e_b)) {
            __syncthreads();
            stage_params(e_ntile, e_b);
            par_ntile = e_ntile; par_img = e_b;
        }
        tick(0);
        chunk_body(0, std::integral_constant<int, 0>{}, std::true_type{}, va, vb);
        if (!(ABL & 2)) __syncthreads();
        chunk_body(1, std::integral_constant<int, 1>{}, std::false_type{}, vb, va);
        if (!(ABL & 2)) __syncthreads();
        for (int c = 2; c < nchunks; c += 2) {
            chunk_body(c, std::integral_constant<int, 0>{}, std::false_type{}, va, vb);
            if (!(ABL & 2)) __syncthreads();
            chunk_body(c + 1, std::integral_constant<int, 1>{}, std::false_type{}, vb, va);
            if (!(ABL & 2)) __syncthreads();
        }
        tick(3);
        cur = nxt; have = have_nxt; in_t = in_n; w_t = w_n;
        if constexpr ((ABL & 32) != 0) {
            f32x4 sacc = acc[0][0];
#pragma unroll
            for (int i = 0; i < NPU; ++i)
#pragma unroll
                for (int nb = 0; nb < NB; ++nb) if (i || nb) sacc += acc[i][nb];
            if (sacc[0] + sacc[1] + sacc[2] + sacc[3] == 123.456f) p.out[tid] = sacc[0];
            continue;
        }
        float* out_b = p.out + (size_t)e_b * (size_t)(p.H + 2) * (p.W + 2 + (p.out_p8 ? 6 : 0)) * p.Cout;
        const float* res_b = nullptr;
        if (EPI & (E_RES | E_RES_UPS)) res_b = p.res + (size_t)e_b * (size_t)(p.Hr + 2) * (p.Wr + 2) * p.Cout;
        const int yb = e_y0 + 4 * tg + 2 * tr, xb = e_x0 + 2 * tc;
        f32x4 resv[NB][2][2];
        if (EPI & (E_RES | E_RES_UPS)) {
#pragma unroll
            for (int nb = 0; nb < NB; ++nb)
#pragma unroll
                for (int i = 0; i < 2; ++i)
#pragma unroll
                    for (int j = 0; j < 2; ++j) {
                        const int y = yb + i, x = xb + j;
                        const int ry = (EPI & E_RES_UPS) ? (y >> 1) : y, rx = (EPI & E_RES_UPS) ? (x >> 1) : x;
                        resv[nb][i][j] = f32x4{0.f, 0.f, 0.f, 0.f};
                        if (y < p.H && x < p.W)
                            resv[nb][i][j] = *(const f32x4*)(res_b + ((ry + 1) * (p.Wr + 2) + rx + 1) * p.Cout + e_ntile * 32 + nb * 16 + 4 * q);
                    }
        }
#pragma unroll
        for (int nb = 0; nb < NB; ++nb) {
            const int co = e_ntile * 32 + nb * 16 + 4 * q;
            f32x4 Y[2][2];
            f32x4 T[2][3];
#pragma unroll
            for (int c = 0; c < 3; ++c) {
                T[0][c] = acc[0 + c][nb] + acc[3 + c][nb];
                T[1][c] = acc[0 + c][nb] + acc[6 + c][nb];
            }
#pragma unroll
            for (int i = 0; i < 2; ++i) {
                Y[i][0] = T[i][0] + T[i][1];
                Y[i][1] = T[i][0] + T[i][2];
            }
            const char* pl = par + (nb * 16 + 4 * q) * 4;
            const f32x4 bias = *(const f32x4*)(pl);
            f32x4 m1, r1, lo1, hi1, m2, r2, lo2, hi2, smean, sstd;
            if (EPI & E_NORM1) {
                m1 = *(const f32x4*)(pl + 128); r1 = *(const f32x4*)(pl + 256);
                lo1 = *(const f32x4*)(pl + 384); hi1 = *(const f32x4*)(pl + 512);
            }
            if (EPI & E_NORM2) {
                m2 = *(const f32x4*)(pl + 640); r2 = *(const f32x4*)(pl + 768);
                lo2 = *(const f32x4*)(pl + 896); hi2 = *(const f32x4*)(pl + 1024);
                smean = *(const f32x4*)(pl + 1152); sstd = *(const f32x4*)(pl + 1280);
            }
#pragma unroll
            for (int i = 0; i < 2; ++i)
#pragma unroll
                for (int j = 0; j < 2; ++j) {
                    const int y = yb + i, x = xb + j;
                    f32x4 o = e4add(Y[i][j], bias);
                    if (EPI & E_RELU) o = f4relu(o);
                    if (EPI & E_LRELU) o = f4lrelu(o);
                    if (EPI & E_NORM1) o = f4norm_clamp(o, m1, r1, lo1, hi1);
                    if (EPI & (E_RES | E_RES_UPS)) o = e4add(o, resv[nb][i][j]);
                    if (EPI & E_NORM2) o = e4fma(f4norm_clamp(o, m2, r2, lo2, hi2), sstd, smean);
                    if (y < p.H && x < p.W) {
                        if (ABL & 4) { if (o[0] == 123.456f) out_b[co] = o[0]; }
                        else if (p.out_p8) *(f32x4*)(out_b + (size_t)(co >> 3) * ((size_t)(p.H + 2) * (p.W + 8) * 8) + ((size_t)(y + 1) * (p.W + 8) + x + 4) * 8 + (co & 7)) = o;
                        else *(f32x4*)(out_b + ((y + 1) * (p.W + 2) + x + 1) * p.Cout + co) = o;
                    }
                }
        }
        tick(5);
    }
    asm volatile("s_waitcnt vmcnt(0)" ::: "memory");
    if ((ABL & 16) && lane == 0) {
        long long* dbg = p.dbg;
#pragma unroll
        for (int k = 0; k < 6; ++k) dbg[(blockIdx.x * NW + wave) * 6 + k] = tl[k];
    }
}

template <int EPI, int ABL = 0, int NW = 4, int UPS = 1, int SC = 0, int PERIMG = 0>
__global__ __launch_bounds__(NW * 64, (SC ? Ups5Geo::OCC : WinoGeo<NW, UPS>::OCC)) void conv_wino_k(const ConvP p) {
    static_assert(UPS == 1 && NW == 4, "library kernel: upsample-fused form, 4 waves");
    if constexpr (SC) conv_ups5_body<EPI, PERIMG>(p);
    else conv_upw_body<EPI, ABL, NW, UPS, PERIMG>(p);
}

__global__ void pack_wino_k(const float* __restrict__ w, float* __restrict__ dst, int Cout, int Cin, int ups) {
    constexpr int CH = 16;
    const int npt = ups ? 9 : 16, pw = ups ? 3 : 4;
    const int np = npt;
    const size_t total = (size_t)Cout * Cin * np;
    for (size_t i = blockIdx.x * (size_t)blockDim.x + threadIdx.x; i < total; i += (size_t)gridDim.x * blockDim.x) {
        size_t r = i;
        const int cl = (int)(r % CH); r /= CH;
        const int j = r & 31; r >>= 5;
        const int pos = (int)(r % np); r /= np;
        const int nchunks = Cin / CH;
        const int chunk = r % nchunks; r /= nchunks;
        const int n_tile = (int)r;
        const int e = cl & 3, qs = cl >> 2;
        const int qq = qs ^ ((0 - (j >> 2)) & 3);
        const int co = n_tile * 32 + j, ci = chunk * CH + qq * 4 + e;
        const float* g = w + ((size_t)co * Cin + ci) * 9;
        const int pr = pos / pw, pc = pos % pw;
        auto G3 = [&](int row, float g0, float g1, float g2) {
            if (ups) return row == 0 ? g0 + g1 + g2 : (row == 1 ? g0 : g2);
            return row == 0 ? g0 : (row == 1 ? 0.5f * (g0 + g1 + g2) : (row == 2 ? 0.5f * (g0 - g1 + g2) : g2));
        };
        float rowv[3];
#pragma unroll
        for (int kx = 0; kx < 3; ++kx) rowv[kx] = G3(pr, g[0 * 3 + kx], g[1 * 3 + kx], g[2 * 3 + kx]);
        dst[i] = G3(pc, rowv[0], rowv[1], rowv[2]);
    }
}
```

Measured before the change: 860.1.

## Reload kernel args via pointer, peel tail chunks, fold wave offset into LDS base

```diff
diff --git a/rerevst-code_amd/csrc/conv_f43.h b/rerevst-code_amd/csrc/conv_f43.h
--- a/rerevst-code_amd/csrc/conv_f43.h
+++ b/rerevst-code_amd/csrc/conv_f43.h
@@ -128,10 +128,12 @@
 #define P8_COL0 4
 #endif
 template <int EPI, int LAY = 0>
-__global__ __launch_bounds__(256, 1) void conv_f43_k(const ConvP p) {
+__global__ __launch_bounds__(256, 1) void conv_f43_k(const ConvP) {
     static_assert(!(EPI & E_RES), "same-resolution residuals are not needed by the layers this kernel serves");
     constexpr bool INP8 = (LAY & 1) != 0, OUTP8 = (LAY & 2) != 0;
-    const int WP = p.Wi + 2 + (INP8 ? P8_PAD : 0);
+    const ConvPK p0 = conv_args();
+    auto wp_of = [](const ConvPK k) { return k->Wi + 2 + (INP8 ? P8_PAD : 0); };
+    const int WP = wp_of(p0);
     using G = F43Geo;
     constexpr int ABL = F43_ABL;
     constexpr int RAW_BYTES = G::RAW_BYTES, U_BYTES = G::U_BYTES, NT = G::NT, NPOS = G::NPOS;
@@ -140,15 +142,16 @@
     const int wave = __builtin_amdgcn_readfirstlane(tid >> 6);
     const int lane = tid & 63, t = lane & 15, q = lane >> 4;
     const int tr = t >> 3, tc = t & 7;
-    const int nchunks = p.Cin >> 3;
-    const int n_ntiles = p.Cout >> 5;
+    const int nchunks = p0->Cin >> 3;
 
     struct Item { int tx, ty, b, nt; };
     Item cur, nxt, dlt;
     {
+        const ConvPK p = p0;
+        const int n_ntiles = p->Cout >> 5;
         const int GD = gridDim.x, w = blockIdx.x;
         int pix, dpix;
-        if (p.xcd_slabs) {
+        if (p->xcd_slabs) {
             const int PT = (GD >> 3) / n_ntiles;
             pix = (w & 7) * PT + (w >> 3) / n_ntiles; dpix = 8 * PT;
             cur.nt = (w >> 3) % n_ntiles; dlt.nt = 0;
@@ -156,32 +159,35 @@
             cur.nt = w % n_ntiles; pix = w / n_ntiles;
             dlt.nt = GD % n_ntiles; dpix = GD / n_ntiles;
         }
-        cur.tx = pix % p.tiles_x; cur.ty = (pix / p.tiles_x) % p.tiles_y; cur.b = pix / (p.tiles_x * p.tiles_y);
-        dlt.tx = dpix % p.tiles_x; dlt.ty = (dpix / p.tiles_x) % p.tiles_y; dlt.b = dpix / (p.tiles_x * p.tiles_y);
+        cur.tx = pix % p->tiles_x; cur.ty = (pix / p->tiles_x) % p->tiles_y; cur.b = pix / (p->tiles_x * p->tiles_y);
+        dlt.tx = dpix % p->tiles_x; dlt.ty = (dpix / p->tiles_x) % p->tiles_y; dlt.b = dpix / (p->tiles_x * p->tiles_y);
     }
-    auto advance = [&](const Item& a) {
+    auto advance = [&](const ConvPK p, const Item& a) {
+        const int n_ntiles = p->Cout >> 5;
         Item r = a;
         r.nt += dlt.nt;
         int carry = 0;
         if (r.nt >= n_ntiles) { r.nt -= n_ntiles; carry = 1; }
         r.tx += dlt.tx + carry;
-        if (r.tx >= p.tiles_x) { r.tx -= p.tiles_x; r.ty += 1; }
+        if (r.tx >= p->tiles_x) { r.tx -= p->tiles_x; r.ty += 1; }
         r.ty += dlt.ty;
-        if (r.ty >= p.tiles_y) { r.ty -= p.tiles_y; r.b += 1; }
+        if (r.ty >= p->tiles_y) { r.ty -= p->tiles_y; r.b += 1; }
         r.b += dlt.b;
         return r;
     };
-    const size_t img_floats = (size_t)(p.Hi + 2) * WP * p.Cin;
-    auto in_of = [&](const Item& a) {
-        return p.in + (size_t)a.b * img_floats + (size_t)(((a.ty + p.ty0) * 32) * WP + (a.tx + p.tx0) * 32 + (INP8 ? P8_COL0 - 1 : 0)) * (INP8 ? 8 : p.Cin);
-    };
-    const size_t plane_floats = (size_t)(p.Hi + 2) * WP * 8;
-    auto lim_of = [&](const Item& a) {
-        const long rows_left = (long)(p.Hi + 2) - (long)(a.ty + p.ty0) * 32;
-        const long n = (rows_left * WP - (long)(a.tx + p.tx0) * 32 - (INP8 ? P8_COL0 - 1 : 0)) * (INP8 ? 8 : p.Cin) * 4;
+    auto in_of = [&](const ConvPK p, const Item& a) {
+        const int WP = wp_of(p);
+        const size_t img_floats = (size_t)(p->Hi + 2) * WP * p->Cin;
+        return p->in + (size_t)a.b * img_floats + (size_t)(((a.ty + p->ty0) * 32) * WP + (a.tx + p->tx0) * 32 + (INP8 ? P8_COL0 - 1 : 0)) * (INP8 ? 8 : p->Cin);
+    };
+    const size_t plane_floats = (size_t)(p0->Hi + 2) * WP * 8;
+    auto lim_of = [&](const ConvPK p, const Item& a) {
+        const int WP = wp_of(p);
+        const long rows_left = (long)(p->Hi + 2) - (long)(a.ty + p->ty0) * 32;
+        const long n = (rows_left * WP - (long)(a.tx + p->tx0) * 32 - (INP8 ? P8_COL0 - 1 : 0)) * (INP8 ? 8 : p->Cin) * 4;
         return (int)(n > 0x7fffffffL ? 0x7fffffffL : n);
     };
-    auto w_of = [&](const Item& a) { return p.wpk + (size_t)a.nt * nchunks * (U_BYTES / 4); };
+    auto w_of = [&](const ConvPK p, const Item& a) { return p->wpk + (size_t)a.nt * nchunks * (U_BYTES / 4); };
     int asrc[G::RAW_IT];
 #pragma unroll
     for (int it = 0; it < G::RAW_IT; ++it) {
@@ -189,13 +195,13 @@
         if (e >= G::RAW_PIECES) e = 0;
         const int half = e & 1, xd = (e >> 1) % 9, ph = ((e >> 1) / 9) & 3, y = (e >> 1) / 36;
         const int x = 4 * xd + ph, par = (y >> 2) & 1;
-        asrc[it] = ((y * WP + x) * (INP8 ? 8 : p.Cin) + 4 * (half ^ par)) * 4;
+        asrc[it] = ((y * WP + x) * (INP8 ? 8 : p0->Cin) + 4 * (half ^ par)) * 4;
         if (ABL & 64) asrc[it] = (it * NT + tid) * 16;
     }
-    bool have = cur.b < p.B, have_nxt = false;
-    const float* in_t = in_of(cur);
-    const float* w_t = w_of(cur);
-    int lim_t = lim_of(cur);
+    bool have = cur.b < p0->B, have_nxt = false;
+    const float* in_t = in_of(p0, cur);
+    const float* w_t = w_of(p0, cur);
+    int lim_t = lim_of(p0, cur);
     const float* in_n = in_t;
     const float* w_n = w_t;
     int lim_n = lim_t;
@@ -213,15 +219,16 @@
     char* const par = smem + 2 * RAW_BYTES + 2 * U_BYTES;
     auto stage_params = [&](int ntile, int img) {
         if (wave < 2) {
+            const ConvPK p = conv_args();
             const int e = tid;
             const int row = e >> 3, col = (e & 7) * 4;
-            const float* src = p.bias;
+            const float* src = p->bias;
             int off = ntile * 32 + col;
-            const int pb = img * p.par_bstride;
-            if (row >= 1 && row <= 4) { src = (EPI & E_NORM1) ? p.n1 : p.bias; off += (EPI & E_NORM1) ? (row - 1) * p.Cout + pb : 0; }
-            if (row >= 5 && row <= 8) { src = (EPI & E_NORM2) ? p.n2 : p.bias; off += (EPI & E_NORM2) ? (row - 5) * p.Cout + pb : 0; }
-            if (row >= 9) { src = (EPI & E_NORM2) ? p.sty : p.bias; off += (EPI & E_NORM2) ? (row - 9) * p.Cout + pb : 0; }
-            if (row > 10) { src = p.bias; off = ntile * 32; }
+            const int pb = img * p->par_bstride;
+            if (row >= 1 && row <= 4) { src = (EPI & E_NORM1) ? p->n1 : p->bias; off += (EPI & E_NORM1) ? (row - 1) * p->Cout + pb : 0; }
+            if (row >= 5 && row <= 8) { src = (EPI & E_NORM2) ? p->n2 : p->bias; off += (EPI & E_NORM2) ? (row - 5) * p->Cout + pb : 0; }
+            if (row >= 9) { src = (EPI & E_NORM2) ? p->sty : p->bias; off += (EPI & E_NORM2) ? (row - 9) * p->Cout + pb : 0; }
+            if (row > 10) { src = p->bias; off = ntile * 32; }
             glds16(src + off, par + wave * 1024);
         }
     };
@@ -232,14 +239,14 @@
     const unsigned rawB = lds0 + y0 * G::RAW_ROW_BYTES + tc * 32 + ((q ^ (2 * ((tr & 1) ^ 1))) << 3);
     const unsigned offU = lds0 + 2 * RAW_BYTES + t * 64 + ((q ^ ((0 - (t >> 2)) & 3)) << 4);
 
-    const unsigned lane_off = (unsigned)(((4 * (q >> 1)) * (p.W + 2) + 16 * (q & 1)) * p.Cout + 2 * t) * 4u;
 #ifndef F43_NAG
 #define F43_NAG 28
 #endif
     constexpr int NAG = F43_NAG;
     f32x4 accA[NAG][2], accV[NPOS - NAG][2];
     int par_ntile = -1, par_img = -1;
-    long long tl[6] = {0, 0, 0, 0, 0, 0}, tl_t = 0;
+    long long tl[10] = {0, 0, 0, 0, 0, 0, 0, 0, 0, 0}, tl_t = 0, pair_t = 0;
+    const long long run_ck = (ABL & 16) ? clock64() : 0, run_rt = (ABL & 16) ? wall_clock64() : 0;
     auto tick = [&](int k) { if (ABL & 16) { const long long n = clock64(); tl[k] += n - tl_t; tl_t = n; } };
     f32x2 v[NPOS];
     f32x4 ur[2][6];
@@ -268,17 +275,22 @@
         }, std::make_integer_sequence<int, 6>{});
     };
 
-    auto chunk_body = [&](int c, auto par_c, auto first_c, bool last) {
+    auto chunk_body = [&](int c, auto par_c, auto first_c, auto tail_c) {
         constexpr int PAR = decltype(par_c)::value;
         constexpr bool FIRST = decltype(first_c)::value;
-        const bool own_u = c + 1 < nchunks, own_r = c + 2 < nchunks;
+        constexpr int TAIL = decltype(tail_c)::value;
+        constexpr bool last = TAIL == 2;
+        constexpr bool own_u = TAIL < 2, own_r = TAIL < 1;
         const rsrc_t rs_u = make_rsrc(own_u ? w_t : w_n);
-        const int rchunk = own_r ? c + 2 : c + 2 - nchunks;
+        const int rchunk = own_r ? c + 2 : TAIL - 1;
         const rsrc_t rs_r = make_rsrc(INP8 ? (own_r ? in_t : in_n) + rchunk * plane_floats : (own_r ? in_t : in_n), own_r ? lim_t : lim_n);
         const int usoff = own_u ? (c + 1) * U_BYTES : 0;
         const int rsoff = INP8 ? 0 : rchunk * 32;
-        char* const udst = smem + 2 * RAW_BYTES + (1 - PAR) * U_BYTES;
-        char* const rdst = smem + PAR * RAW_BYTES;
+        int wb = wave * 1024;
+        asm volatile("" : "+s"(wb));
+        lds_char* const wdst = (lds_char*)smem + wb;
+        lds_char* const udst = wdst + 2 * RAW_BYTES + (1 - PAR) * U_BYTES;
+        lds_char* const rdst = wdst + PAR * RAW_BYTES;
         const unsigned ub = offU + PAR * U_BYTES;
         const unsigned ubn = offU + (1 - PAR) * U_BYTES;
         using RBt = std::integral_constant<int, (1 - PAR) * RAW_BYTES>;
@@ -293,8 +305,8 @@
                 constexpr int step = b * 6 + r;
                 auto dma_req = [&](auto nc) {
                     constexpr int n = decltype(nc)::value;
-                    if constexpr (n < G::RAW_IT) bufld16_rs(rs_r, rdst + (n * NT + wave * 64) * 16, asrc[n], rsoff);
-                    else if constexpr (n < G::RAW_IT + G::U_IT) bufld16_rs(rs_u, udst + ((n - G::RAW_IT) * NT + wave * 64) * 16, tid * 16, usoff + (n - G::RAW_IT) * NT * 16);
+                    if constexpr (n < G::RAW_IT) bufld16_rs(rs_r, rdst + n * NT * 16, asrc[n], rsoff);
+                    else if constexpr (n < G::RAW_IT + G::U_IT) bufld16_rs(rs_u, udst + (n - G::RAW_IT) * NT * 16, tid * 16, usoff + (n - G::RAW_IT) * NT * 16);
                 };
                 {
                     constexpr int SPAN = F43_SPAN, NREQ = G::RAW_IT + G::U_IT;
@@ -345,26 +357,41 @@
     }
     if (ABL & 16) tl_t = clock64();
     while (have) {
-        const int e_y0 = (cur.ty + p.ty0) * 32, e_x0 = (cur.tx + p.tx0) * 32, e_b = cur.b, e_ntile = cur.nt;
-        nxt = advance(cur);
-        have_nxt = nxt.b < p.B;
-        in_n = have_nxt ? in_of(nxt) : in_t;
-        w_n = have_nxt ? w_of(nxt) : w_t;
-        lim_n = have_nxt ? lim_of(nxt) : lim_t;
-        if (par_ntile != e_ntile || (p.par_bstride != 0 && par_img != e_b)) {
+        if (par_ntile != cur.nt || (conv_args()->par_bstride != 0 && par_img != cur.b)) {
             __syncthreads();
-            stage_params(e_ntile, e_b);
-            par_ntile = e_ntile; par_img = e_b;
+            stage_params(cur.nt, cur.b);
+            par_ntile = cur.nt; par_img = cur.b;
         }
         tick(0);
-        chunk_body(0, std::integral_constant<int, 0>{}, std::true_type{}, false);
-        chunk_body(1, std::integral_constant<int, 1>{}, std::false_type{}, false);
-        for (int c = 2; c < nchunks; c += 2) {
-            chunk_body(c, std::integral_constant<int, 0>{}, std::false_type{}, false);
-            chunk_body(c + 1, std::integral_constant<int, 1>{}, std::false_type{}, c + 2 == nchunks);
-        }
+        if (ABL & 16) pair_t = tl_t;
+        using C0 = std::integral_constant<int, 0>; using C1 = std::integral_constant<int, 1>; using C2 = std::integral_constant<int, 2>;
+        chunk_body(0, C0{}, std::true_type{}, C0{});
+        chunk_body(1, C1{}, std::false_type{}, C0{});
+        if (ABL & 16) { tl[6] += tl_t - pair_t; pair_t = tl_t; }
+        for (int c = 2; c + 2 < nchunks; c += 2) {
+            chunk_body(c, C0{}, std::false_type{}, C0{});
+            chunk_body(c + 1, C1{}, std::false_type{}, C0{});
+            if ((ABL & 16) && c == 2) tl[7] += tl_t - pair_t;
+        }
+        const int e_b = cur.b, e_ntile = cur.nt;
+        int e_y0, e_x0;
+        {
+            const ConvPK pn = conv_args();
+            e_y0 = (cur.ty + pn->ty0) * 32; e_x0 = (cur.tx + pn->tx0) * 32;
+            nxt = advance(pn, cur);
+            have_nxt = nxt.b < pn->B;
+            in_n = have_nxt ? in_of(pn, nxt) : in_t;
+            w_n = have_nxt ? w_of(pn, nxt) : w_t;
+            lim_n = have_nxt ? lim_of(pn, nxt) : lim_t;
+        }
+        chunk_body(nchunks - 2, C0{}, std::false_type{}, C1{});
+        chunk_body(nchunks - 1, C1{}, std::false_type{}, C2{});
         cur = nxt; have = have_nxt; in_t = in_n; w_t = w_n; lim_t = lim_n;
         asm volatile("s_nop 15\n\ts_nop 7");
+        const ConvPK p = conv_args();
+        int ln = lane;
+        asm volatile("" : "+v"(ln));
+        const int t = ln & 15, q = ln >> 4;
         auto ACC = [&](int i, int nb) -> f32x4 { return i < NAG ? accA[i][nb] : accV[i - NAG][nb]; };
         if (ABL & 32) {
             f32x4 s = ACC(0, 0);
@@ -372,27 +399,28 @@
             for (int i = 0; i < NPOS; ++i)
 #pragma unroll
                 for (int nb = 0; nb < 2; ++nb) if (i || nb) s += ACC(i, nb);
-            if (s[0] + s[1] + s[2] + s[3] == 123.456f) p.out[tid] = s[0];
+            if (s[0] + s[1] + s[2] + s[3] == 123.456f) p->out[tid] = s[0];
             if (have) next_patch();
             continue;
         }
         const int mr = q >> 1, mc0 = 4 * (q & 1);
         const int yb = e_y0 + 8 * wave + 4 * mr, xb0 = e_x0 + 4 * mc0;
+        const unsigned lane_off = (unsigned)(((4 * (q >> 1)) * (p->W + 2) + 16 * (q & 1)) * p->Cout + 2 * t) * 4u;
         constexpr bool POOL = (EPI & E_POOL) != 0;
-        const int Ho = POOL ? (p.H >> 1) : p.H, Wo = POOL ? (p.W >> 1) : p.W;
+        const int Ho = POOL ? (p->H >> 1) : p->H, Wo = POOL ? (p->W >> 1) : p->W;
         constexpr int OP = OUTP8 ? P8_PAD : 0;
-        char* const sb = OUTP8 ? (char*)(p.out + (size_t)e_b * (size_t)(Ho + 2) * (Wo + 2 + OP) * p.Cout + (size_t)e_ntile * 4 * (size_t)(Ho + 2) * (Wo + 2 + OP) * 8 +
+        char* const sb = OUTP8 ? (char*)(p->out + (size_t)e_b * (size_t)(Ho + 2) * (Wo + 2 + OP) * p->Cout + (size_t)e_ntile * 4 * (size_t)(Ho + 2) * (Wo + 2 + OP) * 8 +
                                          ((size_t)((POOL ? (e_y0 >> 1) + 4 * wave : e_y0 + 8 * wave) + 1) * (Wo + 2 + OP) + (POOL ? (e_x0 >> 1) : e_x0) + P8_COL0) * 8)
-                               : (char*)(p.out + (size_t)e_b * (size_t)(Ho + 2) * (Wo + 2) * p.Cout +
-                                 ((size_t)((POOL ? (e_y0 >> 1) + 4 * wave : e_y0 + 8 * wave) + 1) * (Wo + 2) + (POOL ? (e_x0 >> 1) : e_x0) + 1) * p.Cout + e_ntile * 32);
-        int rowb = (Wo + 2) * p.Cout * 4, pixb = p.Cout * 4;
-        unsigned st_off = POOL ? (unsigned)(((2 * mr) * (Wo + 2) + 2 * mc0) * p.Cout + 2 * t) * 4u : lane_off;
+                               : (char*)(p->out + (size_t)e_b * (size_t)(Ho + 2) * (Wo + 2) * p->Cout +
+                                 ((size_t)((POOL ? (e_y0 >> 1) + 4 * wave : e_y0 + 8 * wave) + 1) * (Wo + 2) + (POOL ? (e_x0 >> 1) : e_x0) + 1) * p->Cout + e_ntile * 32);
+        int rowb = (Wo + 2) * p->Cout * 4, pixb = p->Cout * 4;
+        unsigned st_off = POOL ? (unsigned)(((2 * mr) * (Wo + 2) + 2 * mc0) * p->Cout + 2 * t) * 4u : lane_off;
         if constexpr (OUTP8) {
             const unsigned plane = (unsigned)(Ho + 2) * (Wo + 2 + OP) * 32u;
             rowb = (Wo + 2 + OP) * 32; pixb = 32;
-            st_off = (POOL ? (unsigned)((2 * mr) * (Wo + 2 + OP) + 2 * mc0) : (unsigned)((4 * (q >> 1)) * (p.W + 2 + OP) + 16 * (q & 1))) * 32u + (unsigned)(t >> 2) * plane + (unsigned)(t & 3) * 8u;
-        }
-        const bool interior = e_y0 + 32 <= p.H && e_x0 + 32 <= p.W;
+            st_off = (POOL ? (unsigned)((2 * mr) * (Wo + 2 + OP) + 2 * mc0) : (unsigned)((4 * (q >> 1)) * (p->W + 2 + OP) + 16 * (q & 1))) * 32u + (unsigned)(t >> 2) * plane + (unsigned)(t & 3) * 8u;
+        }
+        const bool interior = e_y0 + 32 <= p->H && e_x0 + 32 <= p->W;
         const char* const pl = par + 8 * t;
         const f32x2 bias = *(const f32x2*)(pl);
         f32x2 n1m, n1r, n1lo, n1hi, n2m, n2r, n2lo, n2hi, smean, sstd;
@@ -403,16 +431,16 @@
         }
         f32x2 rres[4][2][2];
         if constexpr ((EPI & E_RES_UPS) != 0) {
-            const float* const res_b = p.res + (size_t)e_b * (size_t)(p.Hr + 2) * (p.Wr + 2) * p.Cout + e_ntile * 32 + 2 * t;
+            const float* const res_b = p->res + (size_t)e_b * (size_t)(p->Hr + 2) * (p->Wr + 2) * p->Cout + e_ntile * 32 + 2 * t;
 #pragma unroll
             for (int e = 0; e < 4; ++e)
 #pragma unroll
                 for (int a = 0; a < 2; ++a)
 #pragma unroll
                     for (int b2 = 0; b2 < 2; ++b2) {
-                        const bool in = (yb + 2 * a < p.H) && (xb0 + 4 * e + 2 * b2 < p.W);
-                        const int pix = in ? (((yb >> 1) + a + 1) * (p.Wr + 2) + ((xb0 + 4 * e) >> 1) + b2 + 1) : 0;
-                        rres[e][a][b2] = *(const f32x2*)(res_b + (size_t)pix * p.Cout);
+                        const bool in = (yb + 2 * a < p->H) && (xb0 + 4 * e + 2 * b2 < p->W);
+                        const int pix = in ? (((yb >> 1) + a + 1) * (p->Wr + 2) + ((xb0 + 4 * e) >> 1) + b2 + 1) : 0;
+                        rres[e][a][b2] = *(const f32x2*)(res_b + (size_t)pix * p->Cout);
                     }
         }
         float lrk = 0.2f;
@@ -483,7 +511,7 @@
                     } else {
 #pragma unroll
                         for (int i = 0; i < 4; ++i)
-                            if (yb + i < p.H && xb0 + 4 * e + j < p.W) *(f32x2*)(dst + i * rowb) = o[i];
+                            if (yb + i < p->H && xb0 + 4 * e + j < p->W) *(f32x2*)(dst + i * rowb) = o[i];
                     }
                 }
             }
@@ -493,8 +521,9 @@
         tick(5);
     }
     if ((ABL & 16) && lane == 0) {
-#pragma unroll
-        for (int k = 0; k < 6; ++k) p.dbg[(blockIdx.x * 4 + wave) * 6 + k] = tl[k];
+        tl[8] = clock64() - run_ck; tl[9] = wall_clock64() - run_rt;
+#pragma unroll
+        for (int k = 0; k < 10; ++k) conv_args()->dbg[(blockIdx.x * 4 + wave) * 10 + k] = tl[k];
     }
 }
 
diff --git a/rerevst-code_amd/csrc/conv_mfma.h b/rerevst-code_amd/csrc/conv_mfma.h
--- a/rerevst-code_amd/csrc/conv_mfma.h
+++ b/rerevst-code_amd/csrc/conv_mfma.h
@@ -41,6 +41,13 @@
     int out_p8;
 };
 
+typedef const __attribute__((address_space(4))) ConvP* ConvPK;
+__device__ __forceinline__ ConvPK conv_args() {
+    ConvPK k = (ConvPK)__builtin_amdgcn_kernarg_segment_ptr();
+    asm volatile("" : "+s"(k));
+    return k;
+}
+
 template <int BN>
 struct WaveCfg {
     static constexpr int WAVES_N = (BN >= 64) ? 2 : 1;
@@ -71,6 +78,12 @@
     return __builtin_amdgcn_make_buffer_rsrc((void*)base, 0, num_records, 0x00020000);
 #else
     return rsrc_t{};
+#endif
+}
+typedef __attribute__((address_space(3))) char lds_char;
+__device__ __forceinline__ void bufld16_rs(rsrc_t rs, lds_char* lds_wave_base, int voff, int soff) {
+#if defined(__HIP_DEVICE_COMPILE__)
+    __builtin_amdgcn_raw_ptr_buffer_load_lds(rs, (__attribute__((address_space(3))) void*)lds_wave_base, 16, voff, soff, 0, 0);
 #endif
 }
 __device__ __forceinline__ void bufld16_rs(rsrc_t rs, char* lds_wave_base, int voff, int soff) {
diff --git a/rerevst-code_amd/csrc/conv_ups5.h b/rerevst-code_amd/csrc/conv_ups5.h
--- a/rerevst-code_amd/csrc/conv_ups5.h
+++ b/rerevst-code_amd/csrc/conv_ups5.h
@@ -49,7 +49,7 @@
 static_assert(Ups5Geo::row_iter(3) < Ups5Geo::NPOS, "next chunk transformed inside the MFMA loop");
 
 template <int EPI, int PERIMG>
-__device__ __forceinline__ void conv_ups5_body(const ConvP& p) {
+__device__ __forceinline__ void conv_ups5_body() {
     static_assert(!(EPI & (E_POOL | E_RES | E_RES_UPS | E_NORM2)), "conv1 epilogues only: bias, activation, saved-stat normalise");
     using G = Ups5Geo;
     constexpr int RAW_BYTES = G::RAW_BYTES, U_BYTES = G::U_BYTES, NT = G::NT, NB = G::NB, NPOS = G::NPOS, NUB = G::NUB;
@@ -59,15 +59,17 @@
     const int lane = tid & 63, t = lane & 15, q = lane >> 4;
     const int tr = t >> 3, tc = t & 7;
     const int tg = wave;
-    const int nchunks = p.Cin >> 4;
-    const int n_ntiles = p.Cout >> 5;
+    const ConvPK p0 = conv_args();
+    const int nchunks = p0->Cin >> 4;
 
     struct Item { int tx, ty, b, nt; };
     Item cur, nxt, dlt;
     {
+        const ConvPK p = p0;
+        const int n_ntiles = p->Cout >> 5;
         const int GD = gridDim.x, w = blockIdx.x;
         int pix, dpix;
-        if (p.xcd_slabs) {
+        if (p->xcd_slabs) {
             const int PT = (GD >> 3) / n_ntiles;
             pix = (w & 7) * PT + (w >> 3) / n_ntiles; dpix = 8 * PT;
             cur.nt = (w >> 3) % n_ntiles; dlt.nt = 0;
@@ -75,25 +77,26 @@
             cur.nt = w % n_ntiles; pix = w / n_ntiles;
             dlt.nt = GD % n_ntiles; dpix = GD / n_ntiles;
         }
-        cur.tx = pix % p.tiles_x; cur.ty = (pix / p.tiles_x) % p.tiles_y; cur.b = pix / (p.tiles_x * p.tiles_y);
-        dlt.tx = dpix % p.tiles_x; dlt.ty = (dpix / p.tiles_x) % p.tiles_y; dlt.b = dpix / (p.tiles_x * p.tiles_y);
-    }
-    auto advance = [&](const Item& a) {
+        cur.tx = pix % p->tiles_x; cur.ty = (pix / p->tiles_x) % p->tiles_y; cur.b = pix / (p->tiles_x * p->tiles_y);
+        dlt.tx = dpix % p->tiles_x; dlt.ty = (dpix / p->tiles_x) % p->tiles_y; dlt.b = dpix / (p->tiles_x * p->tiles_y);
+    }
+    auto advance = [&](const ConvPK p, const Item& a) {
+        const int n_ntiles = p->Cout >> 5;
         Item r = a;
         r.nt += dlt.nt;
         int carry = 0;
         if (r.nt >= n_ntiles) { r.nt -= n_ntiles; carry = 1; }
         r.tx += dlt.tx + carry;
-        if (r.tx >= p.tiles_x) { r.tx -= p.tiles_x; r.ty += 1; }
+        if (r.tx >= p->tiles_x) { r.tx -= p->tiles_x; r.ty += 1; }
         r.ty += dlt.ty;
-        if (r.ty >= p.tiles_y) { r.ty -= p.tiles_y; r.b += 1; }
+        if (r.ty >= p->tiles_y) { r.ty -= p->tiles_y; r.b += 1; }
         r.b += dlt.b;
         return r;
     };
-    auto in_of = [&](const Item& a) {
-        return p.in + (size_t)a.b * (size_t)(p.Hi + 2) * (p.Wi + 2) * p.Cin + (size_t)(((a.ty + p.ty0) * 16) * (p.Wi + 2) + (a.tx + p.tx0) * 16) * p.Cin;
-    };
-    auto w_of = [&](const Item& a) { return p.wpk + (size_t)a.nt * nchunks * (NUB * 32 * 16); };
+    auto in_of = [&](const ConvPK p, const Item& a) {
+        return p->in + (size_t)a.b * (size_t)(p->Hi + 2) * (p->Wi + 2) * p->Cin + (size_t)(((a.ty + p->ty0) * 16) * (p->Wi + 2) + (a.tx + p->tx0) * 16) * p->Cin;
+    };
+    auto w_of = [&](const ConvPK p, const Item& a) { return p->wpk + (size_t)a.nt * nchunks * (NUB * 32 * 16); };
     int asrc[G::RAW_IT];
 #pragma unroll
     for (int it = 0; it < G::RAW_IT; ++it) {
@@ -103,12 +106,13 @@
         if (P >= G::HALO * G::HALO) P = 0;
         const int hf = P >= G::HALF, rem = P - hf * G::HALF;
         const int hy = rem / 9, hx = 2 * (rem - hy * 9) + hf;
-        asrc[it] = ((hy * (p.Wi + 2) + hx) * p.Cin + 4 * (qq ^ ((hx >> 1) & 3))) * 4;
-    }
+        asrc[it] = ((hy * (p0->Wi + 2) + hx) * p0->Cin + 4 * (qq ^ ((hx >> 1) & 3))) * 4;
+    }
+    const int tid16 = tid * 16;
     const int raw_last_num = ((G::RAW_IT - 1) * NT + wave * 64 < G::PIECES) ? 0x7fffffff : 0;
-    bool have = cur.b < p.B, have_nxt = false;
-    const float* in_t = in_of(cur);
-    const float* w_t = w_of(cur);
+    bool have = cur.b < p0->B, have_nxt = false;
+    const float* in_t = in_of(p0, cur);
+    const float* w_t = w_of(p0, cur);
     const float* in_n = in_t;
     const float* w_n = w_t;
     auto stage_u = [&](int chunk) {
@@ -125,13 +129,17 @@
     char* const par = smem + 2 * RAW_BYTES + 2 * U_BYTES;
     auto stage_params = [&](int ntile, int img) {
         if (wave < 2) {
+            const ConvPK p = conv_args();
             const int e = tid;
             const int row = e >> 3, col = (e & 7) * 4;
-            const float* src = p.bias;
-            const int pb = PERIMG ? img * p.par_bstride : 0;
+            int rrow = tid16;
+            asm volatile("" : "+v"(rrow));
+            rrow >>= 7;
+            const float* src = p->bias;
+            const int pb = PERIMG ? img * p->par_bstride : 0;
             int off = ntile * 32 + col;
-            if (row >= 1 && row <= 4) { src = (EPI & E_NORM1) ? p.n1 : p.bias; off = (EPI & E_NORM1) ? ntile * 32 + col + pb + (row - 1) * p.Cout : off; }
-            if (row > 4) { src = p.bias; off = ntile * 32; }
+            if (row >= 1 && row <= 4) { src = (EPI & E_NORM1) ? p->n1 : p->bias; off = (EPI & E_NORM1) ? ntile * 32 + col + pb + (rrow - 1) * p->Cout : off; }
+            if (row > 4) { src = p->bias; off = ntile * 32; }
             glds16(src + off, par + wave * 1024);
         }
     };
@@ -145,7 +153,6 @@
         offD[dx] = lds0 + P * 64 + ((q ^ ((hx >> 1) & 3)) << 4);
     }
     const unsigned offU = lds0 + 2 * RAW_BYTES + t * 64 + ((q ^ ((0 - (t >> 2)) & 3)) << 4);
-    const unsigned offU1 = offU + U_BYTES;
 
     f32x4 acc[NPOS][NB];
     f32x4 va[16], vb[16];
@@ -156,18 +163,23 @@
     auto col_pass = [&](f32x4 (&d)[16], int dx) { pass(d[dx * 4 + 0], d[dx * 4 + 1], d[dx * 4 + 2], d[dx * 4 + 3]); };
     auto row_pass = [&](f32x4 (&d)[16], int r) { pass(d[0 * 4 + r], d[1 * 4 + r], d[2 * 4 + r], d[3 * 4 + r]); };
 
-    auto chunk_body = [&](int c, auto par_c, auto first_c, f32x4 (&vcur)[16], f32x4 (&vnext)[16]) {
+    auto chunk_body = [&](int c, auto par_c, auto first_c, auto tail_c, f32x4 (&vcur)[16], f32x4 (&vnext)[16]) {
         constexpr int PAR = decltype(par_c)::value;
         constexpr bool FIRST = decltype(first_c)::value;
-        const bool own_u = c + 1 < nchunks, own_r = c + 2 < nchunks;
+        constexpr int TAIL = decltype(tail_c)::value;
+        constexpr bool own_u = TAIL < 2, own_r = TAIL < 1;
         const rsrc_t rs_u = make_rsrc(own_u ? w_t : w_n);
         const rsrc_t rs_r = make_rsrc(own_r ? in_t : in_n);
         const rsrc_t rs_rl = make_rsrc(own_r ? in_t : in_n, raw_last_num);
         const int usoff = own_u ? (c + 1) * U_BYTES : 0;
-        const int rsoff = (own_r ? c + 2 : c + 2 - nchunks) * 64;
-        char* const udst = smem + 2 * RAW_BYTES + (1 - PAR) * U_BYTES;
-        char* const rdst = smem + PAR * RAW_BYTES;
-        const unsigned ub = PAR ? offU1 : offU;
+        const int rsoff = (own_r ? c + 2 : TAIL - 1) * 64;
+        int wb = wave * 1024;
+        asm volatile("" : "+s"(wb));
+        lds_char* const wdst = (lds_char*)smem + wb;
+        lds_char* const udst = wdst + 2 * RAW_BYTES + (1 - PAR) * U_BYTES;
+        lds_char* const rdst = wdst + PAR * RAW_BYTES;
+        unsigned ub = offU;
+        if constexpr (PAR != 0) { asm volatile("" : "+v"(ub)); ub += U_BYTES; }
         constexpr int RB = (1 - PAR) * RAW_BYTES;
         f32x4 u[4][NB];
         f32x4 (&d)[16] = vnext;
@@ -194,8 +206,8 @@
                 }
             }
             __builtin_amdgcn_sched_barrier(0);
-            if constexpr (i < G::U_IT) bufld16_rs(rs_u, udst + (i * NT + wave * 64) * 16, tid * 16, usoff + i * NT * 16);
-            if constexpr (i < G::RAW_IT) bufld16_rs(i == G::RAW_IT - 1 ? rs_rl : rs_r, rdst + (i * NT + wave * 64) * 16, asrc[i], rsoff);
+            if constexpr (i < G::U_IT) bufld16_rs(rs_u, udst + i * NT * 16, tid16, usoff + i * NT * 16);
+            if constexpr (i < G::RAW_IT) bufld16_rs(i == G::RAW_IT - 1 ? rs_rl : rs_r, rdst + i * NT * 16, asrc[i], rsoff);
             const f32x4 vv = vcur[G::vidx(i)];
 #pragma unroll
             for (int s = 0; s < 4; ++s)
@@ -227,33 +239,49 @@
         __syncthreads();
     }
     while (have) {
-        const int e_y0 = (cur.ty + p.ty0) * 32, e_x0 = (cur.tx + p.tx0) * 32, e_b = cur.b, e_ntile = cur.nt;
-        nxt = advance(cur);
-        have_nxt = nxt.b < p.B;
-        in_n = have_nxt ? in_of(nxt) : in_t;
-        w_n = have_nxt ? w_of(nxt) : w_t;
-        if (par_ntile != e_ntile || (PERIMG && par_img != e_b)) {
+        if (par_ntile != cur.nt || (PERIMG && par_img != cur.b)) {
             __syncthreads();
-            stage_params(e_ntile, e_b);
-            par_ntile = e_ntile; par_img = e_b;
-        }
-        chunk_body(0, std::integral_constant<int, 0>{}, std::true_type{}, va, vb);
-        __syncthreads();
-        chunk_body(1, std::integral_constant<int, 1>{}, std::false_type{}, vb, va);
-        __syncthreads();
-        for (int c = 2; c < nchunks; c += 2) {
-            chunk_body(c, std::integral_constant<int, 0>{}, std::false_type{}, va, vb);
+            stage_params(cur.nt, cur.b);
+            par_ntile = cur.nt; par_img = cur.b;
+        }
+        using C0 = std::integral_constant<int, 0>; using C1 = std::integral_constant<int, 1>; using C2 = std::integral_constant<int, 2>;
+        chunk_body(0, C0{}, std::true_type{}, C0{}, va, vb);
+        __syncthreads();
+        chunk_body(1, C1{}, std::false_type{}, C0{}, vb, va);
+        __syncthreads();
+        for (int c = 2; c + 2 < nchunks; c += 2) {
+            chunk_body(c, C0{}, std::false_type{}, C0{}, va, vb);
             __syncthreads();
-            chunk_body(c + 1, std::integral_constant<int, 1>{}, std::false_type{}, vb, va);
+            chunk_body(c + 1, C1{}, std::false_type{}, C0{}, vb, va);
             __syncthreads();
         }
+        const int e_b = cur.b, e_ntile = cur.nt;
+        int e_y0, e_x0;
+        {
+            const ConvPK pn = conv_args();
+            e_y0 = (cur.ty + pn->ty0) * 32; e_x0 = (cur.tx + pn->tx0) * 32;
+            nxt = advance(pn, cur);
+            have_nxt = nxt.b < pn->B;
+            in_n = have_nxt ? in_of(pn, nxt) : in_t;
+            w_n = have_nxt ? w_of(pn, nxt) : w_t;
+        }
+        chunk_body(nchunks - 2, C0{}, std::false_type{}, C1{}, va, vb);
+        __syncthreads();
+        chunk_body(nchunks - 1, C1{}, std::false_type{}, C2{}, vb, va);
+        __syncthreads();
         cur = nxt; have = have_nxt; in_t = in_n; w_t = w_n;
 
-        float* out_b = p.out + (size_t)e_b * (size_t)(p.H + 2) * (p.W + 2 + (p.out_p8 ? 6 : 0)) * p.Cout;
+        const ConvPK p = conv_args();
+        int ln = tid16;
+        asm volatile("" : "+v"(ln));
+        ln = (ln >> 4) & 63;
+        const int t = ln & 15, q = ln >> 4, tr = t >> 3, tc = t & 7;
+        float* out_b = p->out + (size_t)e_b * (size_t)(p->H + 2) * (p->W + 2 + (p->out_p8 ? 6 : 0)) * p->Cout;
         const int yb = e_y0 + 8 * tg + 4 * tr, xb = e_x0 + 4 * tc;
+        __builtin_amdgcn_sched_barrier(0);
         {
             const int ly0 = yb >> 1, lx0 = xb >> 1;
-            float* sc_b = p.sc_out + (size_t)e_b * (size_t)(p.Hi + 2) * (p.Wi + 2) * p.Cout;
+            float* sc_b = p->sc_out + (size_t)e_b * (size_t)(p->Hi + 2) * (p->Wi + 2) * p->Cout;
 #pragma unroll
             for (int nb = 0; nb < NB; ++nb) {
                 const f32x4 s0 = f4sub(acc[25][nb], acc[27][nb]), s1 = e4add(acc[25][nb], acc[27][nb]);
@@ -264,8 +292,8 @@
 #pragma unroll
                     for (int b = 0; b < 2; ++b) {
                         const int ly = ly0 + a, lx = lx0 + b;
-                        if (ly < p.Hi && lx < p.Wi)
-                            *(f32x4*)(sc_b + ((size_t)(ly + 1) * (p.Wi + 2) + lx + 1) * p.Cout + e_ntile * 32 + nb * 16 + 4 * q) = sc[a][b];
+                        if (ly < p->Hi && lx < p->Wi)
+                            *(f32x4*)(sc_b + ((size_t)(ly + 1) * (p->Wi + 2) + lx + 1) * p->Cout + e_ntile * 32 + nb * 16 + 4 * q) = sc[a][b];
                     }
             }
         }
@@ -300,9 +328,9 @@
                     if (EPI & E_RELU) o = f4relu(o);
                     if (EPI & E_LRELU) o = f4lrelu(o);
                     if (EPI & E_NORM1) o = f4norm_clamp(o, m1, r1, lo1, hi1);
-                    if (y < p.H && x < p.W) {
-                        if (p.out_p8) *(f32x4*)(out_b + (size_t)(co >> 3) * ((size_t)(p.H + 2) * (p.W + 8) * 8) + ((size_t)(y + 1) * (p.W + 8) + x + 4) * 8 + (co & 7)) = o;
-                        else *(f32x4*)(out_b + ((size_t)(y + 1) * (p.W + 2) + x + 1) * p.Cout + co) = o;
+                    if (y < p->H && x < p->W) {
+                        if (p->out_p8) *(f32x4*)(out_b + (size_t)(co >> 3) * ((size_t)(p->H + 2) * (p->W + 8) * 8) + ((size_t)(y + 1) * (p->W + 8) + x + 4) * 8 + (co & 7)) = o;
+                        else *(f32x4*)(out_b + ((size_t)(y + 1) * (p->W + 2) + x + 1) * p->Cout + co) = o;
                     }
                 }
         }
diff --git a/rerevst-code_amd/csrc/conv_wino.h b/rerevst-code_amd/csrc/conv_wino.h
--- a/rerevst-code_amd/csrc/conv_wino.h
+++ b/rerevst-code_amd/csrc/conv_wino.h
@@ -448,7 +448,7 @@
 template <int EPI, int ABL = 0, int NW = 4, int UPS = 1, int SC = 0, int PERIMG = 0>
 __global__ __launch_bounds__(NW * 64, (SC ? Ups5Geo::OCC : WinoGeo<NW, UPS>::OCC)) void conv_wino_k(const ConvP p) {
     static_assert(UPS == 1 && NW == 4, "library kernel: upsample-fused form, 4 waves");
-    if constexpr (SC) conv_ups5_body<EPI, PERIMG>(p);
+    if constexpr (SC) conv_ups5_body<EPI, PERIMG>();
     else conv_upw_body<EPI, ABL, NW, UPS, PERIMG>(p);
 }
 
```

Measured after the change: 873.7, median of 6. 1.6% higher.
